# byteowlz/kokorox

Hardware: AMD Instinct MI355X
Metric: real-time factor (audio-s/wall-s), 24 kHz, batch=64 (higher is better)
Workload: dtype f32 in / out, f32 accumulate; products on split operands: f16f8 (a_hi b_hi on f16 MFMAs, the cross terms a_lo b_hi + a_hi b_lo of the 7 / 11-tap convs on e4m3 scaled MFMAs: ~17 significant bits per product; every other conv f16x3: ~22) -- wider than the bf16 BASELINE configs[2] names, inside the 1e-; 1 GPU; batch=64/GPU synthetic 128-phoneme utterances (T=130), durations pinned 3,3,3,4 -> F=422 frames = 10.55 s each, noise on, inputs in HBM; batch_per_gpu=64, frames=422, parallelism=utterance-sharded x1, one-time weight broadcast

## Files before the change

kokorox_amd/build.py:

```python
from __future__ import annotations

import os
import subprocess
import sys

HERE = os.path.dirname(os.path.abspath(__file__))
CSRC = os.path.join(HERE, "csrc")
LIB_DIR = os.path.join(HERE, "lib")
LIB_PATH = os.path.join(LIB_DIR, "libkokorox_hip.so")
TEST_LIB_PATH = os.path.join(LIB_DIR, "libkokorox_hip_test.so")
TEST_SOURCES = ["test_hooks.hip"]
SOURCES = ["conv_plan.hip", "conv_mfma.hip", "conv_f16x3.hip", "conv_f16x3_da.hip", "conv_f16x3_da_p1.hip", "conv_f16x3_da_w2.hip", "conv_f16x3_da_s16.hip", "conv_f16x3_da_f8.hip", "conv_f16x3_da_pre.hip", "conv_f16x3_pre.hip", "conv_f16x3_dapn.hip", "conv_f16x3_dag.hip", "kernels_misc.hip", "model.hip", "api.hip", "dispatcher.hip", "onnx_import.cpp"]
HEADERS = ["kx_common.h", "kx_error.h", "conv_epilogue.h", "conv_f16x3_common.h"]
_PUB = os.path.join("..", "..", "include", "kokorox_hip.h")
_PUB_TEST = os.path.join("..", "..", "include", "kokorox_hip_test.h")
EXTRA_DEPS = {"model.hip": ["onnx_import.h", "model.h", _PUB], "api.hip": ["model.h", "kx_handle.h", "api_guard.h", _PUB],
              "dispatcher.hip": ["model.h", "kx_handle.h", "dispatcher_core.h", _PUB],
              "test_hooks.hip": ["model.h", "kx_handle.h", "api_guard.h", _PUB, _PUB_TEST], "onnx_import.cpp": ["onnx_import.h"], "conv_f16x3_da_p1.hip": ["conv_f16x3_da.hip"], "conv_f16x3_da_w2.hip": ["conv_f16x3_da.hip"], "conv_f16x3_da_s16.hip": ["conv_f16x3_da.hip"], "conv_f16x3_da_f8.hip": ["conv_f16x3_da.hip"], "conv_f16x3_da_pre.hip": ["conv_f16x3_da.hip"]}
FLAGS = ["-O3", "--offload-arch=gfx950", "-fPIC", "-std=c++17", "-Wall", "-Wno-unused-result"]


def _hipcc() -> str:
    for cand in (os.environ.get("HIPCC"), "/opt/rocm/bin/hipcc", "hipcc"):
        if cand and (os.path.isabs(cand) and os.path.exists(cand) or not os.path.isabs(cand)):
            return cand
    return "hipcc"


def _newer(target: str, deps) -> bool:
    if not os.path.exists(target):
        return False
    t = os.path.getmtime(target)
    return all(os.path.getmtime(d) <= t for d in deps)


LAST_BUILD = {"compiled": [], "reused": [], "linked": False}


def build_library(force: bool = False, verbose: bool = False) -> str:
    LAST_BUILD["compiled"], LAST_BUILD["reused"], LAST_BUILD["linked"] = [], [], False
    os.makedirs(LIB_DIR, exist_ok=True)
    hdrs = [os.path.join(CSRC, h) for h in HEADERS]
    objs, test_objs, jobs = [], [], []
    for src in SOURCES + TEST_SOURCES:
        s = os.path.join(CSRC, src)
        o = os.path.join(LIB_DIR, os.path.splitext(src)[0] + ".o")
        (test_objs if src in TEST_SOURCES else objs).append(o)
        if force or not _newer(o, [s] + hdrs + [os.path.join(CSRC, d) for d in EXTRA_DEPS.get(src, [])]):
            flags = [f for f in FLAGS if not f.startswith("--offload-arch")] if src.endswith(".cpp") else FLAGS
            jobs.append([_hipcc(), *flags, "-c", s, "-o", o])
            LAST_BUILD["compiled"].append(src)
        else:
            LAST_BUILD["reused"].append(src)
    if jobs:
        from concurrent.futures import ThreadPoolExecutor

        def run(cmd):
            if verbose:
                print(" ".join(cmd), file=sys.stderr)
            subprocess.run(cmd, check=True)

        with ThreadPoolExecutor(max_workers=min(4, len(jobs))) as ex:
            list(ex.map(run, jobs))
    if force or not _newer(LIB_PATH, objs):
        cmd = [_hipcc(), "--offload-arch=gfx950", "-shared", "-fPIC", *objs, "-lpthread", "-o", LIB_PATH]
        if verbose:
            print(" ".join(cmd), file=sys.stderr)
        subprocess.run(cmd, check=True)
        LAST_BUILD["linked"] = True
    if force or not _newer(TEST_LIB_PATH, test_objs + [LIB_PATH]):
        cmd = [_hipcc(), "--offload-arch=gfx950", "-shared", "-fPIC", *test_objs, "-L" + LIB_DIR, "-lkokorox_hip", "-Wl,-rpath,$ORIGIN",
               "-lpthread", "-o", TEST_LIB_PATH]
        if verbose:
            print(" ".join(cmd), file=sys.stderr)
        subprocess.run(cmd, check=True)
    return LIB_PATH


if __name__ == "__main__":
    print(build_library(force="--force" in sys.argv, verbose=True))
```

kokorox_amd/csrc/conv_f16x3.hip:

```cpp
#include "conv_f16x3_common.h"

namespace kx {

template <int BM, int BN, int WM, int WN, int ACT, int TK, bool PF, int VT>
__global__ __launch_bounds__(WM * WN * 64, (WM * WN == 8) ? 4 : ((BM / WM / 32) * (BN / WN / 32) > 6 ? 2 : 3))
void conv1d_f16x3_kernel(const ConvArgs a) {
    constexpr int MT = BM / WM / 32;
    constexpr int NT = BN / WN / 32;
    constexpr int NWV = WM * WN;
    static_assert((NWV == 4 || NWV == 8) && MT >= 1 && NT >= 1, "4 or 8 waves per workgroup");
    static_assert(VT == 1 || (VT <= TK && PF), "virtual taps need TK >= VT and the prefetching build");
    extern __shared__ __attribute__((aligned(16))) unsigned char smem16[];

    const int tid = threadIdx.x;
    const int lane = tid & 63;
    const int wave = __builtin_amdgcn_readfirstlane(tid >> 6);
    const int wm = wave / WN, wn = wave % WN;
    const int r = lane & 31, h = lane >> 5;
    const int b = blockIdx.z, ct = blockIdx.y;
    int tile_x = blockIdx.x;
    if (a.xcd_swizzle && gridDim.x >= 16) {
        const int nx = gridDim.x;
        const int off = (int)(((long)nx * (blockIdx.y + (long)gridDim.y * blockIdx.z)) & 7);
        const int cls = (blockIdx.x + off) & 7;
// ... 223 lines not shown
                half8 al_[2][MT], bh[2][NT], ah[MT], bl[NT];
                load_P(0, al_[0], bh[0]);
#pragma unroll
                for (int tt = 0; tt < TK; ++tt) {
                    if (tt < taps) {
                        load_Q(tt, ah, bl);
#pragma unroll
                        for (int mt = 0; mt < MT; ++mt)
#pragma unroll
                            for (int nt = 0; nt < NT; ++nt)
                                acc[mt][nt] = __builtin_amdgcn_mfma_f32_32x32x16_f16(al_[tt & 1][mt], bh[tt & 1][nt], acc[mt][nt], 0, 0, 0);
                        if (tt + 1 < TK && tt + 1 < taps) load_P(tt + 1, al_[(tt + 1) & 1], bh[(tt + 1) & 1]);
#pragma unroll
                        for (int mt = 0; mt < MT; ++mt)
#pragma unroll
                            for (int nt = 0; nt < NT; ++nt) {
                                acc[mt][nt] = __builtin_amdgcn_mfma_f32_32x32x16_f16(ah[mt], bl[nt], acc[mt][nt], 0, 0, 0);
                                acc[mt][nt] = __builtin_amdgcn_mfma_f32_32x32x16_f16(ah[mt], bh[tt & 1][nt], acc[mt][nt], 0, 0, 0);
                            }
                    }
                }
            }
            unsigned long long tp0 = 0;
            if (a.stamps) tp0 = __builtin_amdgcn_s_memrealtime();
            if (pc + 1 == n_pieces && more)
                asm volatile("s_waitcnt lgkmcnt(0)\n\ts_barrier" ::: "memory");
            else
                __syncthreads();
            if (a.stamps) acc_pbar += __builtin_amdgcn_s_memrealtime() - tp0;
            cur ^= 1;
        }
        if (more) {
            unsigned long long ta = 0, tb = 0;
            if (a.stamps) ta = __builtin_amdgcn_s_memrealtime();
            if (!(a.dbg & 1)) stage_chunk(ch + 1, true);
            if (a.stamps) tb = __builtin_amdgcn_s_memrealtime();
            __syncthreads();
            if (a.stamps) {
                acc_stage += tb - ta;
                acc_bar += __builtin_amdgcn_s_memrealtime() - tb;
            }
        }
    }

    if (a.stamps) st2 = __builtin_amdgcn_s_memrealtime();
    if (a.dbg & 8) return;
    float2* stat_scr = (BM >= 64 || PF) ? reinterpret_cast<float2*>(smem16) + wave * (32 * 33) : nullptr;
    conv_store_tile<MT, NT, EPI_ROWS, (VT > 1)>(a, acc, a.w_unscale, b, ct * BM + wm * (MT * 32), t0 + wn * (NT * 32), r, h, ncols, Lout,
                            tile_x * WN + wn, stat_scr);
    if (a.stamps && tid == 0) {
        const unsigned lin = blockIdx.x + gridDim.x * (blockIdx.y + gridDim.y * blockIdx.z);
        unsigned long long* o = a.stamps + (unsigned long long)lin * 8;
        o[0] = st0; o[1] = st1; o[2] = st2;
        __builtin_amdgcn_s_waitcnt(0);
        o[3] = __builtin_amdgcn_s_memrealtime();
        o[4] = __builtin_amdgcn_s_getreg(63492);
        o[5] = __builtin_readcyclecounter() - cyc0;
        o[6] = acc_stage;
        o[7] = acc_bar | (acc_pbar << 32);
    }
}

int conv16_cu_count() {
    if (const int part = cu_count_override()) return part;
    static std::atomic<int> n[KX_MAX_DEVICES];
    int dev = 0;
    KX_HIP(hipGetDevice(&dev));
    if (dev < 0 || dev >= KX_MAX_DEVICES) return 256;
    int v = n[dev].load(std::memory_order_relaxed);
    if (v == 0) {
        hipDeviceProp_t pr;
        KX_HIP(hipGetDeviceProperties(&pr, dev));
        v = pr.multiProcessorCount > 0 ? pr.multiProcessorCount : 256;
        n[dev].store(v, std::memory_order_relaxed);
    }
    return v;
}

template <int BM, int BN, int WM, int WN, int ACT, int TK, bool PF, int VT = 1>
static void launch_inst16_pf(const ConvArgs& a, int B, int max_cols, hipStream_t s) {
    static DynLdsLimit lds_limit;
    auto kern = conv1d_f16x3_kernel<BM, BN, WM, WN, ACT, TK, PF, VT>;
    const int XW = (BN - 1) * a.stride + (a.K - 1) * a.dil + 1;
    const int XWp = PF ? ((VT > 1) ? 128 : BN + 128) : ((XW + 3) & ~3);
    KX_REQUIRE(!PF || (a.stride == 1 && XW <= XWp), "conv1d f16x3: the prefetching build needs stride 1 and a window <= BN + 128");
    const size_t lds = 16 * ((size_t)2 * TK * 4 * BM + (size_t)VT * 4 * XWp);
    KX_REQUIRE(lds <= 160 * 1024, "conv1d f16x3: LDS tile too large for this k/stride");
    KX_REQUIRE(VT == 1 || (a.K == 1 && a.stride == 1 && XW <= 128), "conv1d f16x3: virtual taps need a k=1 GEMM");
    lds_limit.ensure(reinterpret_cast<const void*>(kern), lds);
    dim3 grid((max_cols + BN - 1) / BN, (a.Cout + BM - 1) / BM, a.merge_T > 0 ? 1 : B);
    KX_REQUIRE(grid.x > 0 && grid.y > 0 && grid.y < 65536 && B > 0 && B < 65536, "conv1d f16x3: bad grid");
    KX_REQUIRE(a.merge_T == 0 || (PF && a.K == 1 && a.stride == 1 && a.pad == 0 && !a.in_up2 && !a.nmean &&
                                  a.store != ST_UPSCATTER && !a.stat_part),
               "conv1d f16x3: merged columns need a plain k=1 GEMM");
    hipLaunchKernelGGL(kern, grid, dim3(WM * WN * 64), lds, s, a);
    KX_HIP(hipGetLastError());
}

template <int BM, int BN, int WM, int WN, int ACT>
static void launch_inst16_act(const ConvPlan& p, const ConvArgs& a, int B, hipStream_t s) {
    if (p.pf)
        launch_inst16_pf<BM, BN, WM, WN, ACT, 3, true>(a, B, p.cols, s);
    else
        launch_inst16_pf<BM, BN, WM, WN, ACT, 3, false>(a, B, p.cols, s);
}

template <int BM, int BN, int WM, int WN>
static void launch_inst16(const ConvPlan& p, const ConvArgs& a, int B, hipStream_t s) {
    if (p.act == ACT_SNAKE)
        launch_inst16_act<BM, BN, WM, WN, ACT_SNAKE>(p, a, B, s);
    else if (p.act == ACT_LEAKY)
        launch_inst16_act<BM, BN, WM, WN, ACT_LEAKY>(p, a, B, s);
    else
        launch_inst16_act<BM, BN, WM, WN, ACT_NONE>(p, a, B, s);
}

static void launch_lds(const ConvPlan& p, const ConvArgs& a, int B, hipStream_t s) {
    if (p.vt > 1) {
        KX_REQUIRE(p.bm == 128 && p.bn == 128 && p.pf && p.act != ACT_SNAKE && (p.vt == 2 || p.vt == 3), "conv1d f16x3: no such virtual-tap form");
        if (p.vt == 3) {
            if (p.act == ACT_LEAKY)
                launch_inst16_pf<128, 128, 2, 2, ACT_LEAKY, 3, true, 3>(a, B, p.cols, s);
            else
                launch_inst16_pf<128, 128, 2, 2, ACT_NONE, 3, true, 3>(a, B, p.cols, s);
        } else {
            if (p.act == ACT_LEAKY)
                launch_inst16_pf<128, 128, 2, 2, ACT_LEAKY, 2, true, 2>(a, B, p.cols, s);
            else
                launch_inst16_pf<128, 128, 2, 2, ACT_NONE, 2, true, 2>(a, B, p.cols, s);
        }
        return;
    }
    const int bm = p.bm, bn = p.bn, wm = p.wm, wn = p.wn;
    if (bm == 128 && bn == 128 && wm == 4 && wn == 1)
        launch_inst16<128, 128, 4, 1>(p, a, B, s);
    else if (bm == 128 && bn == 128 && wm == 2 && wn == 2)
        launch_inst16<128, 128, 2, 2>(p, a, B, s);
    else if (bm == 128 && bn == 256 && wm == 2 && wn == 2)
        launch_inst16<128, 256, 2, 2>(p, a, B, s);
    else if (bm == 64 && bn == 256 && wm == 1 && wn == 4)
        launch_inst16<64, 256, 1, 4>(p, a, B, s);
    else if (bm == 32 && bn == 256 && wm == 1 && wn == 4)
        launch_inst16<32, 256, 1, 4>(p, a, B, s);
    else
        throw Error(1, "conv1d f16x3: no such LDS-DMA form");
}

void launch_conv(const ConvPlan& p, const ConvArgs& a, int B, hipStream_t s) {
    if (p.form == FORM_F32) {
        launch_conv1d(a, p.bm, B, p.cols, s);
        return;
    }
    KX_REQUIRE(a.n_chunks16 == (a.Cin + CK16 - 1) / CK16 && a.w16 != nullptr, "conv1d f16x3: weights not packed");
    KX_REQUIRE(a.epi != EPI_GELU_NEW || p.vt > 1 || p.form == FORM_DAG || p.form == FORM_DAGN,
               "conv1d f16x3: gelu epilogue exists only for k=1 GEMMs with >= 48 input channels");
    KX_REQUIRE(p.merged == (a.merge_T > 0), "conv1d f16x3: merged columns do not match the plan");
    if (p.cols <= 0) return;
    switch (p.form) {
        case FORM_LDS: launch_lds(p, a, B, s); return;
        case FORM_DAG:
        case FORM_DAGN: launch_conv1d_f16x3_dag(p, a, B, s); return;
        case FORM_DAPN: launch_conv1d_f16x3_dapn(a, B, p.cols, s); return;
        case FORM_DA_PRE: launch_conv16_da_pre(p, a, B, s); return;
        case FORM_DA_S16: launch_conv16_da_s16(p, a, B, s); return;
        case FORM_DA_F8: launch_conv16_da_f8(p, a, B, s); return;
        case FORM_DA:
            if (p.p1) {
                launch_conv16_da_p1(p, a, B, s);
                return;
            }
            [[fallthrough]];
        case FORM_DA_W2: {
            static const int dephase = getenv("KX_DEPHASE") ? atoi(getenv("KX_DEPHASE")) : 0;
            static const int dephase_mode = getenv("KX_DEPHASE_MODE") ? atoi(getenv("KX_DEPHASE_MODE")) : 1;
            ConvArgs d;
            const ConvArgs* ap = &a;
            if (dephase > 0 && p.bn == 256) {
                d = a;
                const long grid_n = (long)((p.cols + 255) / 256) * ((a.Cout + 127) / 128) * B;
                const double tile_cycles = (double)a.n_chunks16 * a.K * 8 * 96 * 2.5 + 50000.0;
                d.dephase_cycles = grid_n >= 1024 ? (int)(tile_cycles * dephase / 1000.0) : 0;
                d.dephase_mode = dephase_mode;
                ap = &d;
            }
            if (p.form == FORM_DA_W2)
                launch_conv16_da_w2(p, *ap, B, s);
            else
                launch_conv16_da(p, *ap, B, s);
            return;
        }
    }
    throw Error(1, "conv1d: unknown kernel form");
}

size_t packed_conv16_halves(int rows, int Cin, int K, int BM) {
    const size_t tiles = (rows + BM - 1) / BM, chunks = (Cin + CK16 - 1) / CK16;
    return tiles * chunks * K * 4 * BM * 8;
}

__global__ void absmax_kernel(const float* p, long n, unsigned* out) {
    float m = 0.f;
    for (long i = blockIdx.x * (long)blockDim.x + threadIdx.x; i < n; i += (long)gridDim.x * blockDim.x)
        m = fmaxf(m, fabsf(p[i]));
    for (int o = 32; o > 0; o >>= 1) m = fmaxf(m, __shfl_down(m, o));
    if ((threadIdx.x & 63) == 0) atomicMax(out, __float_as_uint(m));
}

float device_absmax(const float* p, long n, hipStream_t s) {
    unsigned* d;
    KX_HIP(hipMalloc((void**)&d, 4));
    KX_HIP(hipMemsetAsync(d, 0, 4, s));
    const int blocks = (int)((n + 255) / 256 < 1024 ? (n + 255) / 256 : 1024);
    hipLaunchKernelGGL(absmax_kernel, dim3(blocks), dim3(256), 0, s, p, n, d);
    unsigned hbits = 0;
    KX_HIP(hipMemcpyAsync(&hbits, d, 4, hipMemcpyDeviceToHost, s));
    KX_HIP(hipStreamSynchronize(s));
    KX_HIP(hipFree(d));
    float f;
    memcpy(&f, &hbits, 4);
    return f;
}

int pick_weight_shift(float absmax) {
    if (!(absmax > 0.f) || !std::isfinite(absmax)) return 0;
    int e;
    frexpf(absmax, &e);
    int ws = 12 - e;
    if (ws < -8) ws = -8;
    if (ws > 24) ws = 24;
    return ws;
}

__global__ void pack_conv16_kernel(PackSrc src, _Float16* dst, int Cout, int Cin, int K, int BM, float wscale,
                                   long total_pairs) {
    const int n_chunks = (Cin + CK16 - 1) / CK16;
    for (long e = blockIdx.x * (long)blockDim.x + threadIdx.x; e < total_pairs; e += (long)gridDim.x * blockDim.x) {
        long q = e;
        const int j8 = q % 8; q /= 8;
        const int m = q % BM; q /= BM;
        const int hh = q % 2; q /= 2;
        const int tap = q % K; q /= K;
        const int ch = q % n_chunks; q /= n_chunks;
        const int co = (int)q * BM + m, ci = ch * CK16 + hh * 8 + j8;
        float v = 0.f;
        if (co < Cout && ci < Cin) {
            int rr = co;
            const float* p = src.p[0];
            if (rr >= src.rows[0]) { rr -= src.rows[0]; p = src.p[1];
                if (rr >= src.rows[1]) { rr -= src.rows[1]; p = src.p[2]; } }
            v = p[((long)rr * Cin + ci) * K + tap] * wscale;
        }
        const _Float16 hi = (_Float16)v;
        const _Float16 lo = (_Float16)(v - (float)hi);
        const long base = ((((long)q * n_chunks + ch) * K + tap) * 2) * 2 * BM * 8;
        dst[base + ((0 * 2 + hh) * (long)BM + m) * 8 + j8] = hi;
        dst[base + ((1 * 2 + hh) * (long)BM + m) * 8 + j8] = lo;
    }
}

void launch_pack_conv16(const PackSrc& src, void* dst, int Cout, int Cin, int K, int BM, float wscale, hipStream_t s) {
    const long total = (long)packed_conv16_halves(Cout, Cin, K, BM) / 2;
    const int blocks = (int)((total + 255) / 256 < 4096 ? (total + 255) / 256 : 4096);
    hipLaunchKernelGGL(pack_conv16_kernel, dim3(blocks), dim3(256), 0, s, src, static_cast<_Float16*>(dst), Cout, Cin, K,
                       BM, wscale, total);
    KX_HIP(hipGetLastError());
}

__global__ void pack_convT16_kernel(const float* w, _Float16* dst, int Cin, int Cout, int sd, int BM, float wscale,
                                    long total_pairs) {
    const int n_chunks = (Cin + CK16 - 1) / CK16;
    const int rows = sd * Cout, k = 2 * sd;
    for (long e = blockIdx.x * (long)blockDim.x + threadIdx.x; e < total_pairs; e += (long)gridDim.x * blockDim.x) {
        long q = e;
        const int j8 = q % 8; q /= 8;
        const int m = q % BM; q /= BM;
        const int hh = q % 2; q /= 2;
        const int tap = q % 2; q /= 2;
        const int ch = q % n_chunks; q /= n_chunks;
        const int row = (int)q * BM + m, ci = ch * CK16 + hh * 8 + j8;
        float v = 0.f;
        if (row < rows && ci < Cin) {
            const int sdiv = sd, co = row / sdiv, p = row % sdiv;
            v = w[((long)ci * Cout + co) * k + (tap == 0 ? p + sd : p)] * wscale;
        }
        const _Float16 hi = (_Float16)v;
        const _Float16 lo = (_Float16)(v - (float)hi);
        const long base = ((((long)q * n_chunks + ch) * 2 + tap) * 2) * 2 * BM * 8;
        dst[base + ((0 * 2 + hh) * (long)BM + m) * 8 + j8] = hi;
        dst[base + ((1 * 2 + hh) * (long)BM + m) * 8 + j8] = lo;
    }
}

__global__ void image_to_bf16_kernel(const _Float16* src, unsigned short* dst, long n_halves, int plane) {
    for (long e = blockIdx.x * (long)blockDim.x + threadIdx.x; e < n_halves; e += (long)gridDim.x * blockDim.x) {
        const long blk = e / (2 * plane), in_blk = e - blk * 2 * plane;
        if (in_blk >= plane) {
            dst[e] = 0;
            continue;
        }
        const float v = (float)src[e] + (float)src[e + plane];
        unsigned u = __float_as_uint(v);
        u += 0x7fffu + ((u >> 16) & 1u);
        dst[e] = (unsigned short)(u >> 16);
    }
}
void launch_image_to_bf16(const void* w16, void* dst, size_t n_halves, hipStream_t s) {
    const int plane = 2 * 128 * 8;
    const int blocks = (int)((n_halves + 255) / 256 < 4096 ? (n_halves + 255) / 256 : 4096);
    hipLaunchKernelGGL(image_to_bf16_kernel, dim3(blocks), dim3(256), 0, s, static_cast<const _Float16*>(w16), static_cast<unsigned short*>(dst),
                       (long)n_halves, plane);
    KX_HIP(hipGetLastError());
}

size_t packed_conv8x_bytes(int rows, int Cin, int K) {
// ... 46 lines not shown
```

kokorox_amd/csrc/conv_plan.hip:

```cpp
#include "kx_common.h"

namespace kx {

static bool da_eligible(int BM, int K, int dil, int stride, bool merged) {
    return BM == 128 && stride == 1 && !merged && (K - 1) * dil + 256 <= 384;
}

static bool f8_taps(int K, int dil) { return (K == 11 || K == 7 || K == 3) && (K - 1) * dil <= 64; }

static bool s16_shape(int BM, int K, int dil, int stride, int act, int n_chunks16, bool merged, int pmode) {
    const bool taps = K == 11 || (K == 7 && dil == 1) || (pmode == 2 && f8_taps(K, dil));
    return BM == 128 && stride == 1 && !merged && pmode != 1 && act == ACT_SNAKE && taps && (K - 1) * dil <= 64 && n_chunks16 >= 2 &&
           (n_chunks16 & 1) == 0;
}

bool conv16_f8_layer(int BM, int rows, int K, int n_chunks16) {
    return BM == 128 && f8_taps(K, 1) && (K != 3 || rows <= 256) && n_chunks16 >= 2 && (n_chunks16 & 1) == 0;
}

ConvPlan conv_plan(const ConvLaunch& c) {
    ConvPlan p{};
    p.bm = c.BM;
    p.act = c.act;
    p.vt = 1;
    p.cols = c.cols;
    const bool stats = c.stats && c.store == ST_NORMAL && !c.accum;
    auto set_stats = [&](int stat_cols) {
        if (!stats) return;
        p.stat_cols = stat_cols;
        p.stat_tiles = (p.cols + p.bn - 1) / p.bn * (p.bn / stat_cols);
    };
    if (c.mode == CONV_F32) {
        p.form = FORM_F32;
        p.bn = c.BM == 128 ? 128 : 256;
        set_stats(64);
        return p;
    }
    const int route = c.force & 3;
    const int pmode = c.prec1 ? 1 : (c.f8 ? 2 : 0);

    const bool pre_form = c.stride == 1 && c.K >= 2 && !c.in_up2 && c.act != ACT_SNAKE && !c.prec1 &&
                          da_eligible(c.BM, c.K, c.dil, c.stride, false);
    p.pre = (c.mode == CONV_F16X3 || c.mode == CONV_F16F8) && c.image && pre_form && (c.image == 2 || c.rows >= 512);

    p.merged = c.B > 1 && c.K == 1 && c.stride == 1 && c.pad == 0 && !c.in_up2 && !c.norm && c.store != ST_UPSCATTER && !c.stats &&
               c.merge_T > 0 && c.merge_T <= 512;
    if (p.merged) p.cols = c.B * c.merge_T;

    if (c.BM != 128) {
        p.form = FORM_LDS;
        p.bn = 256;
        p.wm = 1;
        p.wn = 4;
        p.pf = c.stride == 1 && (c.K - 1) * c.dil <= 128;
        set_stats(64);
        return p;
    }

    if (c.K == 1 && c.stride == 1 && !stats && !c.in_up2 && c.n_chunks16 >= 3 && c.act != ACT_SNAKE) {
        const long tiles = (long)((p.cols + 127) / 128) * ((c.rows + 127) / 128);
        if (route != FORCE_LDS && !c.norm && c.store != ST_UPSCATTER) {
            const long wgs = tiles * (p.merged ? 1 : c.B);
            const bool narrow_ok = (c.x_bs * c.B + 16L * c.x_ld) * 4 < (1L << 31);
            p.form = narrow_ok && 2 * wgs <= c.cus ? FORM_DAGN : FORM_DAG;
            p.bn = p.form == FORM_DAGN ? 32 : 128;
            return p;
        }
        p.form = FORM_LDS;
        p.bn = 128;
        p.wm = 2;
        p.wn = 2;
        p.pf = 1;
        p.vt = tiles > 2L * c.cus ? 2 : 3;
        return p;
    }

    const bool da = route != FORCE_LDS && da_eligible(c.BM, c.K, c.dil, c.stride, p.merged);
    const bool small = (long)((p.cols + 255) / 256) * ((c.rows + 127) / 128) * c.B < 256;
    if (route != FORCE_LDS && !(c.force & FORCE_NO_S16) && s16_shape(c.BM, c.K, c.dil, c.stride, c.act, c.n_chunks16, p.merged, pmode)) {
        p.form = pmode == 2 ? FORM_DA_F8 : FORM_DA_S16;
        p.kt = c.K;
        p.bn = small && route != FORCE_DA ? 128 : 192;
        set_stats(64);
    } else if (!da || (route != FORCE_DA && c.cols <= 160 && !stats)) {
        p.form = FORM_LDS;
        const bool short_seq = c.cols <= 160 && !stats;
        p.bn = !short_seq && !small ? 256 : 128;
        p.wm = !short_seq && small ? 4 : 2;
        p.wn = !short_seq && small ? 1 : 2;
        p.pf = c.stride == 1 && (c.K - 1) * c.dil <= 128;
        set_stats(p.bn / p.wn);
    } else {
        p.bn = small && route != FORCE_DA ? 128 : 256;
        set_stats(128);
        const bool w64 = (c.K - 1) * c.dil <= 64;
        if (p.pre) {
            const bool narrow = p.bn == 128 && !c.prec1 && c.rows % 32 == 0 && c.K <= 12 && c.epi == EPI_NONE &&
                                (c.store == ST_NORMAL || c.store == ST_UPSCATTER) && (long)c.n_chunks16 * c.K < 5000;
            p.form = narrow ? FORM_DAPN : FORM_DA_PRE;
            p.act = ACT_NONE;
            p.kt = c.K == 3 && w64 ? 3 : 0;
        } else {
            const bool unrolled = w64 && ((c.act == ACT_SNAKE && (c.K == 11 || c.K == 7 || c.K == 3)) || (c.act == ACT_LEAKY && c.K == 3));
            p.kt = unrolled ? c.K : 0;
            p.p1 = c.prec1 != 0;
            p.bf = c.prec1 == 2;
            p.form = unrolled && p.bn == 256 && !c.prec1 && !(c.force & FORCE_DA_4X1) ? FORM_DA_W2 : FORM_DA;
        }
    }
    const bool flat_form = p.form != FORM_LDS;
    p.flat_bn = flat_form && c.B > 1 && p.cols > 0 ? p.bn : 0;
    return p;
}

}
```

kokorox_amd/csrc/kernels_misc.hip:

```cpp
#include <cmath>

#include <atomic>

#include "kx_common.h"

namespace kx {

__device__ __forceinline__ int len_of(const LenMap& m, int b) { return m.lens[b] * m.mul + m.add; }

__global__ void vec_add_kernel(const float* a, const float* b, float* out, int n) {
    int i = blockIdx.x * blockDim.x + threadIdx.x;
    if (i < n) out[i] = a[i] + (b ? b[i] : 0.f);
}
void launch_vec_add(const float* a, const float* b, float* out, int n, hipStream_t s) {
    hipLaunchKernelGGL(vec_add_kernel, dim3((n + 255) / 256), dim3(256), 0, s, a, b, out, n);
    KX_HIP(hipGetLastError());
}

__global__ void transpose_whh_kernel(const float* w, float* out) {
    int i = blockIdx.x * blockDim.x + threadIdx.x;
    if (i < 1024 * 256) {
        int r = i / 256, k = i % 256;
        out[((k >> 2) * 1024 + r) * 4 + (k & 3)] = w[i];
    }
}
void launch_transpose_whh(const float* whh, float* out, hipStream_t s) {
    hipLaunchKernelGGL(transpose_whh_kernel, dim3(1024), dim3(256), 0, s, whh, out);
    KX_HIP(hipGetLastError());
}

__device__ __forceinline__ long checked_id(long id, int n_vocab, int b, int t, unsigned* bad) {
    if (id >= 0 && id < n_vocab) return id;
    if (bad) atomicCAS(bad, 0u, (((unsigned)b << 16) | (unsigned)t) + 1u);
    return id < 0 ? 0 : n_vocab - 1;
}

__global__ void albert_embed_kernel(const int64_t* ids, long ids_stride, const float* word, const float* type0,
                                    const float* pos, float* out, long bs, int ld, const int* lens, int n_vocab,
                                    unsigned* bad) {
    const int t = blockIdx.x, b = blockIdx.y, e = threadIdx.x;
    if (t >= lens[b]) return;
    const long id = checked_id(ids[b * ids_stride + t], n_vocab, b, t, e == 0 ? bad : nullptr);
    out[b * bs + (long)e * ld + t] = (word[id * 128 + e] + type0[e]) + pos[t * 128 + e];
}
void launch_albert_embed(const int64_t* ids, long ids_stride, const float* word, const float* type0,
                         const float* pos, float* out, long bs, int ld, const int* lens, int B, int Tmax,
                         int n_vocab, unsigned* bad_id, hipStream_t s) {
    hipLaunchKernelGGL(albert_embed_kernel, dim3(Tmax, B), dim3(128), 0, s, ids, ids_stride, word, type0, pos,
                       out, bs, ld, lens, n_vocab, bad_id);
    KX_HIP(hipGetLastError());
}

__global__ void embed_kernel(const int64_t* ids, long ids_stride, const float* table, int C, float* out, long bs,
                             int ld, const int* lens, int n_vocab, unsigned* bad) {
    const int t = blockIdx.x, b = blockIdx.y;
    if (t >= lens[b]) return;
    const long id = checked_id(ids[b * ids_stride + t], n_vocab, b, t, threadIdx.x == 0 ? bad : nullptr);
    for (int c = threadIdx.x; c < C; c += blockDim.x) out[b * bs + (long)c * ld + t] = table[id * C + c];
}
void launch_embed(const int64_t* ids, long ids_stride, const float* table, int C, float* out, long bs, int ld,
                  const int* lens, int B, int Tmax, int n_vocab, unsigned* bad_id, hipStream_t s) {
    hipLaunchKernelGGL(embed_kernel, dim3(Tmax, B), dim3(256), 0, s, ids, ids_stride, table, C, out, bs, ld, lens,
                       n_vocab, bad_id);
    KX_HIP(hipGetLastError());
}

template <int CPT>
__global__ __launch_bounds__(1024) void layernorm_ch_kernel(const float* x, float* y, long bs, int ld, int C,
                                                            LenMap len, float eps, int mode, const float* g,
                                                            const float* be, int g_bs, float leaky) {
    __shared__ float red[2][16][16];
    const int tx = threadIdx.x & 15, cg = threadIdx.x >> 4, wave = threadIdx.x >> 6;
    const bool wave_lead = (threadIdx.x & 63) < 16;
    const int b = blockIdx.y, t = blockIdx.x * 16 + tx;
    const int L = len_of(len, b);
    const bool ok = t < L;
    const float* xb = x + b * bs + (ok ? t : 0);
    float v[CPT];
    float s = 0.f;
#pragma unroll
    for (int i = 0; i < CPT; ++i) {
        const int c = cg + 64 * i;
        v[i] = (ok && c < C) ? xb[(long)c * ld] : 0.f;
        s += v[i];
    }
    s += __shfl_xor(s, 16);
    s += __shfl_xor(s, 32);
    if (wave_lead) red[0][wave][tx] = s;
    __syncthreads();
    float tot = 0.f;
#pragma unroll
    for (int k = 0; k < 16; ++k) tot += red[0][k][tx];
    const float mean = tot / (float)C;
    float q = 0.f;
#pragma unroll
    for (int i = 0; i < CPT; ++i) {
        const int c = cg + 64 * i;
        const float d = (c < C) ? v[i] - mean : 0.f;
        q += d * d;
    }
    q += __shfl_xor(q, 16);
    q += __shfl_xor(q, 32);
    if (wave_lead) red[1][wave][tx] = q;
    __syncthreads();
    float qt = 0.f;
#pragma unroll
    for (int k = 0; k < 16; ++k) qt += red[1][k][tx];
    const float rstd = 1.0f / sqrtf(qt / (float)C + eps);
    if (!ok) return;
    float* yb = y + b * bs + t;
#pragma unroll
    for (int i = 0; i < CPT; ++i) {
        const int c = cg + 64 * i;
        if (c >= C) continue;
        float o = (v[i] - mean) * rstd;
        if (mode == LN_AFFINE)
            o = o * g[c] + be[c];
        else if (mode == LN_ADA)
            o = (1.0f + g[(long)b * g_bs + c]) * o + be[(long)b * g_bs + c];
        if (leaky != 0.f) o = o > 0.f ? o : o * leaky;
        yb[(long)c * ld] = o;
    }
}
void launch_layernorm_ch(const float* x, float* y, long bs, int ld, int C, LenMap len, int B, int Lmax, float eps,
                         int mode, const float* g, const float* be, int g_bs, float leaky, hipStream_t s) {
    if (Lmax <= 0) return;
    KX_REQUIRE(C <= 768, "layernorm: at most 768 channels");
    const dim3 grid((Lmax + 15) / 16, B), block(1024);
    if (C <= 128)
        hipLaunchKernelGGL(layernorm_ch_kernel<2>, grid, block, 0, s, x, y, bs, ld, C, len, eps, mode, g, be, g_bs, leaky);
    else if (C <= 512)
        hipLaunchKernelGGL(layernorm_ch_kernel<8>, grid, block, 0, s, x, y, bs, ld, C, len, eps, mode, g, be, g_bs, leaky);
    else
        hipLaunchKernelGGL(layernorm_ch_kernel<12>, grid, block, 0, s, x, y, bs, ld, C, len, eps, mode, g, be, g_bs, leaky);
    KX_HIP(hipGetLastError());
}

__global__ __launch_bounds__(256) void attention_mfma_kernel(const float* qkv, long bs, int ld, float* ctx, long cbs,
                                                             int cld, const int* lens) {
    using f32x16 = __attribute__((ext_vector_type(16))) float;
    const int b = blockIdx.x, hd = blockIdx.y;
    const int lane = threadIdx.x & 63, wave = threadIdx.x >> 6;
    const int i = lane & 31, hh = lane >> 5;
    const int T = lens[b];
    const int q0 = (blockIdx.z * 4 + wave) * 32;
    if (q0 >= T) return;
    const float* Q = qkv + b * bs + (long)(hd * 64) * ld;
    const float* Kp = Q + (long)768 * ld;
    const float* V = Q + (long)1536 * ld;
    const int qi = q0 + i < T ? q0 + i : T - 1;
    float qreg[32];
#pragma unroll
    for (int s = 0; s < 32; ++s) qreg[s] = Q[(long)(2 * s + hh) * ld + qi];
    f32x16 o0, o1;
#pragma unroll
    for (int e = 0; e < 16; ++e) o0[e] = o1[e] = 0.f;
    float mrun = -INFINITY, lrun = 0.f;
    for (int k0 = 0; k0 < T; k0 += 32) {
        const int kj = k0 + i < T ? k0 + i : T - 1;
        f32x16 st;
#pragma unroll
        for (int e = 0; e < 16; ++e) st[e] = 0.f;
#pragma unroll
        for (int s = 0; s < 32; ++s)
            st = __builtin_amdgcn_mfma_f32_32x32x2f32(Kp[(long)(2 * s + hh) * ld + kj], qreg[s], st, 0, 0, 0);
        float bm = -INFINITY;
#pragma unroll
        for (int e = 0; e < 16; ++e) {
            const int j = k0 + (e & 3) + 8 * (e >> 2) + 4 * hh;
            st[e] = j < T ? st[e] * 0.125f : -INFINITY;
            bm = fmaxf(bm, st[e]);
        }
        bm = fmaxf(bm, __shfl_xor(bm, 32));
        const float mn = fmaxf(mrun, bm);
        const float alpha = expf(mrun - mn);
        float psum = 0.f;
#pragma unroll
        for (int e = 0; e < 16; ++e) {
            st[e] = expf(st[e] - mn);
            psum += st[e];
        }
        psum += __shfl_xor(psum, 32);
        lrun = lrun * alpha + psum;
        mrun = mn;
#pragma unroll
        for (int e = 0; e < 16; ++e) {
            o0[e] *= alpha;
            o1[e] *= alpha;
        }
#pragma unroll
        for (int dt = 0; dt < 2; ++dt) {
            const float* vrow = V + (long)(dt * 32 + i) * ld + k0 + 4 * hh;
            float vv[16];
#pragma unroll
            for (int g4 = 0; g4 < 4; ++g4) {
                const float4 v4 = *reinterpret_cast<const float4*>(vrow + 8 * g4);
                const int j = k0 + 8 * g4 + 4 * hh;
                vv[4 * g4 + 0] = j + 0 < T ? v4.x : 0.f;
                vv[4 * g4 + 1] = j + 1 < T ? v4.y : 0.f;
                vv[4 * g4 + 2] = j + 2 < T ? v4.z : 0.f;
                vv[4 * g4 + 3] = j + 3 < T ? v4.w : 0.f;
            }
#pragma unroll
            for (int s = 0; s < 16; ++s) {
                if (dt == 0)
                    o0 = __builtin_amdgcn_mfma_f32_32x32x2f32(vv[s], st[s], o0, 0, 0, 0);
                else
                    o1 = __builtin_amdgcn_mfma_f32_32x32x2f32(vv[s], st[s], o1, 0, 0, 0);
            }
        }
    }
    if (q0 + i < T) {
        const float inv = 1.0f / lrun;
        float* cb = ctx + b * cbs + (long)(hd * 64) * cld + q0 + i;
#pragma unroll
        for (int e = 0; e < 16; ++e) {
            const int d = (e & 3) + 8 * (e >> 2) + 4 * hh;
            cb[(long)d * cld] = o0[e] * inv;
            cb[(long)(32 + d) * cld] = o1[e] * inv;
        }
    }
}

void launch_attention(const float* qkv, long bs, int ld, float* ctx, long cbs, int cld, const int* lens, int B,
                      int Tmax, hipStream_t s) {
    KX_REQUIRE(Tmax <= 512, "attention: T > 512");
    KX_REQUIRE(ld % 32 == 0 && ld >= ((Tmax + 31) & ~31), "attention: rows must be padded to a multiple of 32 columns");
    hipLaunchKernelGGL(attention_mfma_kernel, dim3(B, 12, (Tmax + 127) / 128), dim3(256), 0, s, qkv, bs, ld, ctx, cbs,
                       cld, lens);
    KX_HIP(hipGetLastError());
}

__global__ __launch_bounds__(256) void style_fc_kernel(const FcDesc* desc, const float* styles, float* out,
                                                       long out_bs) {
    __shared__ float sv[128];
    const FcDesc d = desc[blockIdx.x];
    const int b = blockIdx.y;
    if (threadIdx.x < 128) sv[threadIdx.x] = styles[b * 256 + d.style_off + threadIdx.x];
    __syncthreads();
    for (int o = threadIdx.x; o < d.n_out; o += 256) {
        const float4* wr = reinterpret_cast<const float4*>(d.w + (long)o * 128);
        float acc = 0.f;
#pragma unroll 8
        for (int k = 0; k < 32; ++k) {
            const float4 w4 = wr[k];
            acc += w4.x * sv[4 * k] + w4.y * sv[4 * k + 1] + w4.z * sv[4 * k + 2] + w4.w * sv[4 * k + 3];
        }
        out[b * out_bs + d.out_off + o] = acc + d.b[o];
    }
}
__global__ void tile_prefix_kernel(LenMap len, int extra, int bn, int B, int* out) {
    if (threadIdx.x != 0 || blockIdx.x != 0) return;
    int acc = 0;
    for (int b = 0; b < B; ++b) {
        out[b] = acc;
        const int cols = len.lens[b] * len.mul + len.add + extra;
        acc += cols > 0 ? (cols + bn - 1) / bn : 0;
    }
    out[B] = acc;
}

void launch_tile_prefix(LenMap len, int extra, int bn, int B, int* out, hipStream_t s) {
    hipLaunchKernelGGL(tile_prefix_kernel, dim3(1), dim3(64), 0, s, len, extra, bn, B, out);
    KX_HIP(hipGetLastError());
}

void launch_style_fc(const FcDesc* d_desc, int n_desc, const float* styles, float* out, long out_bs, int B,
                     hipStream_t s) {
    hipLaunchKernelGGL(style_fc_kernel, dim3(n_desc, B), dim3(256), 0, s, d_desc, styles, out, out_bs);
    KX_HIP(hipGetLastError());
}

__global__ __launch_bounds__(256) void in_stats_kernel(const float* x, long bs, int ld, LenMap len, const float* gb,
                                                       long gb_bs, int C, float* mean, float* scale, float* shift,
                                                       int n_bs, float2* raw_out) {
    __shared__ double rs[4], rq[4];
    const int c = blockIdx.x, b = blockIdx.y;
    const int L = len_of(len, b);
    const float* row = x + b * bs + (long)c * ld;
    double s = 0.0, q = 0.0;
    const int L4 = L & ~3;
    const float4* row4 = reinterpret_cast<const float4*>(row);
    int t = threadIdx.x;
    for (; 4 * (t + 256) < L4; t += 512) {
        const float4 u = row4[t], w = row4[t + 256];
        const double a0 = u.x, a1 = u.y, a2 = u.z, a3 = u.w, b0 = w.x, b1 = w.y, b2 = w.z, b3 = w.w;
        s += ((a0 + a1) + (a2 + a3)) + ((b0 + b1) + (b2 + b3));
        q += ((a0 * a0 + a1 * a1) + (a2 * a2 + a3 * a3)) + ((b0 * b0 + b1 * b1) + (b2 * b2 + b3 * b3));
    }
    for (; 4 * t < L4; t += 256) {
        const float4 u = row4[t];
        const double a0 = u.x, a1 = u.y, a2 = u.z, a3 = u.w;
        s += (a0 + a1) + (a2 + a3);
        q += (a0 * a0 + a1 * a1) + (a2 * a2 + a3 * a3);
    }
    for (int e = L4 + threadIdx.x; e < L; e += 256) {
        const double v = (double)row[e];
        s += v;
        q += v * v;
    }
    for (int o = 32; o > 0; o >>= 1) {
        s += __shfl_down(s, o);
        q += __shfl_down(q, o);
    }
    const int lane = threadIdx.x & 63, wave = threadIdx.x >> 6;
    if (lane == 0) {
        rs[wave] = s;
        rq[wave] = q;
    }
    __syncthreads();
    if (threadIdx.x == 0) {
        const double S = (rs[0] + rs[1]) + (rs[2] + rs[3]), Q = (rq[0] + rq[1]) + (rq[2] + rq[3]);
        if (raw_out) {
            const float sh = (float)S, qh = (float)Q;
            raw_out[((long)b * C + c) * 2 + 0] = make_float2(sh, qh);
            raw_out[((long)b * C + c) * 2 + 1] = make_float2((float)(S - (double)sh), (float)(Q - (double)qh));
        }
        const double m = L > 0 ? S / L : 0.0;
        double var = L > 0 ? Q / L - m * m : 0.0;
        if (var < 0.0) var = 0.0;
        const float rstd = (float)(1.0 / sqrt(var + 1e-5));
        const float g = gb[b * gb_bs + c], be = gb[b * gb_bs + C + c];
        mean[(long)b * n_bs + c] = (float)m;
        scale[(long)b * n_bs + c] = (1.0f + g) * rstd;
        shift[(long)b * n_bs + c] = be;
    }
}
void launch_in_stats(const float* x, long bs, int ld, int C, LenMap len, int B, const float* gb, long gb_bs,
                     float* mean, float* scale, float* shift, int n_bs, float2* raw_out, hipStream_t s) {
    hipLaunchKernelGGL(in_stats_kernel, dim3(C, B), dim3(256), 0, s, x, bs, ld, len, gb, gb_bs, C, mean, scale,
                       shift, n_bs, raw_out);
    KX_HIP(hipGetLastError());
}

__global__ __launch_bounds__(64) void stats_finalize_kernel(const float2* part, int tiles, int cols_per_tile, int C,
                                                            LenMap len, const float* gb, long gb_bs, float* mean,
                                                            float* scale, float* shift, int n_bs) {
    const int c = blockIdx.x, b = blockIdx.y;
    const int L = len_of(len, b);
    const int used = ((L + cols_per_tile - 1) / cols_per_tile);
    const float2* p = part + ((long)b * C + c) * tiles;
    double s = 0.0, q = 0.0;
    for (int i = threadIdx.x; i < used && i < tiles; i += 64) {
        const float2 v = p[i];
        s += (double)v.x;
        q += (double)v.y;
    }
    for (int o = 32; o > 0; o >>= 1) {
        s += __shfl_down(s, o);
        q += __shfl_down(q, o);
    }
    if (threadIdx.x == 0) {
        const double m = L > 0 ? s / L : 0.0;
        double var = L > 0 ? q / L - m * m : 0.0;
        if (var < 0.0) var = 0.0;
        const float rstd = (float)(1.0 / sqrt(var + 1e-5));
        const float g = gb[b * gb_bs + c], be = gb[b * gb_bs + C + c];
        mean[(long)b * n_bs + c] = (float)m;
        scale[(long)b * n_bs + c] = (1.0f + g) * rstd;
        shift[(long)b * n_bs + c] = be;
    }
}
void launch_stats_finalize(const float2* part, int tiles, int cols_per_tile, int C, LenMap len, int B, const float* gb,
                           long gb_bs, float* mean, float* scale, float* shift, int n_bs, hipStream_t s) {
    hipLaunchKernelGGL(stats_finalize_kernel, dim3(C, B), dim3(64), 0, s, part, tiles, cols_per_tile, C, len, gb, gb_bs,
                       mean, scale, shift, n_bs);
    KX_HIP(hipGetLastError());
}

__global__ void style_mix_kernel(const float* table, int n_voices, const int* voice_ids, const float* weights,
                                 int max_mix, const int* rows, const int* kinds, float* styles) {
#pragma clang fp contract(off)
    const int b = blockIdx.x, j = threadIdx.x;
    const int kind = kinds ? kinds[b] : (max_mix == 1 ? 1 : 2);
    if (kind == 0) return;
    const int row = rows[b];
    const int* v = voice_ids + (long)b * max_mix;
    const float* w = weights + (long)b * max_mix;
    float acc = 0.f;
    if (kind == 1) {
        acc = table[((long)v[0] * 511 + row) * 256 + j];
    } else {
// ... 776 lines not shown
```

kokorox_amd/csrc/kx_common.h:

```cpp
#pragma once
#include <hip/hip_runtime.h>

#include <cmath>
#include <cstdint>
#include <cstring>
#include <cstdio>
#include <stdexcept>
#include <string>

#include <atomic>
#include <mutex>

#include "kx_error.h"

namespace kx {

constexpr int KX_MAX_DEVICES = 64;

struct DynLdsLimit {
    std::atomic<size_t> limit[KX_MAX_DEVICES];
    std::mutex mu;
    DynLdsLimit() {
        for (auto& l : limit) l.store(64 * 1024);
    }
    void ensure(const void* kern, size_t lds) {
        int dev = 0;
        if (hipGetDevice(&dev) != hipSuccess || dev < 0 || dev >= KX_MAX_DEVICES) throw Error(3, "dynamic LDS limit: bad current device");
        if (lds <= limit[dev].load(std::memory_order_acquire)) return;
        std::lock_guard<std::mutex> lk(mu);
        if (lds <= limit[dev].load(std::memory_order_relaxed)) return;
        const hipError_t e = hipFuncSetAttribute(kern, hipFuncAttributeMaxDynamicSharedMemorySize, (int)lds);
        if (e != hipSuccess) throw Error(3, std::string("hipFuncSetAttribute(MaxDynamicSharedMemorySize): ") + hipGetErrorString(e));
        limit[dev].store(lds, std::memory_order_release);
    }
};

#define KX_HIP(expr)                                                                       \
    do {                                                                                   \
        hipError_t e_ = (expr);                                                            \
        if (e_ != hipSuccess)                                                              \
            throw kx::Error(3, std::string(#expr) + ": " + hipGetErrorString(e_) + " (" +  \
                                   __FILE__ + ":" + std::to_string(__LINE__) + ")");       \
    } while (0)

#define KX_REQUIRE(cond, msg)                                 \
    do {                                                      \
        if (!(cond)) throw kx::Error(1, std::string(msg));    \
    } while (0)

struct LenMap {
    const int* lens;
    int mul, add;
};

constexpr int CONV_CK = 8;

enum ConvAct { ACT_NONE = 0, ACT_LEAKY = 1, ACT_SNAKE = 2 };
enum ConvStore { ST_NORMAL = 0, ST_TMAJOR = 1, ST_UPSCATTER = 2 };
enum ConvEpi { EPI_NONE = 0, EPI_GELU_NEW = 1 };

struct ConvArgs {
    const float* x;
    long x_bs;
    int x_ld;
    int Cin;
    LenMap in_len;
    LenMap out_len;
    const float* w;
    const float* bias;
    const float* nmean;
    const float* nscale;
    const float* nshift;
    int n_bs;
    int act;
    float slope;
    const float* alpha;
    int K, dil, stride, pad;
    int in_up2;
    int Cout;
    int n_chunks;
    float* y;
    long y_bs;
    int y_ld;
    const float* resid;
    long r_bs;
    int r_ld;
    int accum;
    float out_mul;
    float out_div;
    int epi;
    int store;
    int up_s, up_pad, up_off, up_reflect, up_cout;
    const void* w16;
    const void* w16b;
    const void* w8x;
    int epi_stream;
    int n_chunks16;
    float w_unscale;
    float x_prescale;
    int merge_T;
    int merge_B;
    float2* stat_part;
    int stat_tiles;
    int xcd_swizzle;
    int ws_force;
    unsigned long long* stamps;
    int prec1;
    int dephase_cycles, dephase_mode;
    int dbg;
    const int* tile_prefix;
    int flat_ny;
    int flat_B;
    int flat_tiles_host, flat_bn_host;
    const void* x16;
    long x16_bs;
    int x16_ld;
};

enum ConvMode { CONV_F32 = 0, CONV_F16X3 = 1, CONV_F16X3_LDS = 2, CONV_F16X3_DA = 3, CONV_F16 = 4, CONV_BF16 = 5, CONV_F16F8 = 6 };
enum ConvForm {
    FORM_F32 = 0,
    FORM_LDS,
    FORM_DAG,
    FORM_DAGN,
    FORM_DA,
    FORM_DA_W2,
    FORM_DA_S16,
    FORM_DA_F8,
    FORM_DA_PRE,
    FORM_DAPN,
};
enum ConvForce { FORCE_LDS = 1, FORCE_DA = 2, FORCE_DA_4X1 = 4, FORCE_NO_S16 = 8 };

struct ConvLaunch {
    int mode;
    int prec1;
    int f8;
    int BM, rows, n_chunks16, K, dil, stride, pad, act, in_up2, store, accum, epi;
    int norm;
    int stats;
    int image;
    int merge_T;
    long x_bs;
    int x_ld;
    int B, cols;
    int cus;
    int force;
};
struct ConvPlan {
    int form;
    int bm, act, kt, wm, wn, vt, pf, p1, bf;
    int bn;
    int cols;
    int merged;
    int pre;
    int stat_cols, stat_tiles;
    int flat_bn;
};
ConvPlan conv_plan(const ConvLaunch& c);
bool conv16_f8_layer(int BM, int rows, int K, int n_chunks16);
void launch_conv(const ConvPlan& p, const ConvArgs& a, int B, hipStream_t s);
int conv16_cu_count();
int cu_count_override();

size_t conv16_pre_image_bytes(int Cin, int x_ld);
void launch_split_image(const ConvArgs& a, int B, int Lmax, void* img, long img_bs, hipStream_t s);

void launch_tile_prefix(LenMap len, int extra, int bn, int B, int* out, hipStream_t s);

inline int conv_pick_bm(int rows) { return rows >= 128 ? 128 : (rows > 32 ? 64 : 32); }

void launch_conv1d(const ConvArgs& a, int BM, int B, int max_cols, hipStream_t s);

struct PackSrc {
    const float* p[3];
    int rows[3];
};
void launch_pack_conv(const PackSrc& src, float* dst, int Cout, int Cin, int K, int BM, hipStream_t s);
void launch_pack_convT(const float* w, float* dst, int Cin, int Cout, int s, int BM, hipStream_t s_);
size_t packed_conv_floats(int rows, int Cin, int K, int BM);

void launch_conv16_da(const ConvPlan& p, const ConvArgs& a, int B, hipStream_t s);
void launch_conv16_da_p1(const ConvPlan& p, const ConvArgs& a, int B, hipStream_t s);
void launch_conv16_da_w2(const ConvPlan& p, const ConvArgs& a, int B, hipStream_t s);
void launch_conv16_da_s16(const ConvPlan& p, const ConvArgs& a, int B, hipStream_t s);
void launch_conv16_da_f8(const ConvPlan& p, const ConvArgs& a, int B, hipStream_t s);
void launch_conv16_da_pre(const ConvPlan& p, const ConvArgs& a, int B, hipStream_t s);
void launch_conv1d_f16x3_dapn(const ConvArgs& a, int B, int max_cols, hipStream_t s);
void launch_conv1d_f16x3_dag(const ConvPlan& p, const ConvArgs& a, int B, hipStream_t s);
size_t packed_conv16_halves(int rows, int Cin, int K, int BM);
float device_absmax(const float* p, long n, hipStream_t s);
int pick_weight_shift(float absmax);
void launch_pack_conv16(const PackSrc& src, void* dst, int Cout, int Cin, int K, int BM, float wscale, hipStream_t s);
void launch_pack_convT16(const float* w, void* dst, int Cin, int Cout, int sd, int BM, float wscale, hipStream_t s);
void launch_image_to_bf16(const void* w16, void* dst, size_t n_halves, hipStream_t s);
size_t packed_conv8x_bytes(int rows, int Cin, int K);
void launch_pack_conv8x(const void* w16, void* dst, int rows, int Cin, int K, hipStream_t s);

void launch_vec_add(const float* a, const float* b, float* out, int n, hipStream_t s);
void launch_transpose_whh(const float* whh, float* out, hipStream_t s);

void launch_albert_embed(const int64_t* ids, long ids_stride, const float* word, const float* type0,
                         const float* pos, float* out, long bs, int ld, const int* lens, int B, int Tmax,
                         int n_vocab, unsigned* bad_id, hipStream_t s);
void launch_embed(const int64_t* ids, long ids_stride, const float* table, int C, float* out, long bs, int ld,
                  const int* lens, int B, int Tmax, int n_vocab, unsigned* bad_id, hipStream_t s);

enum LnMode { LN_PLAIN = 0, LN_AFFINE = 1, LN_ADA = 2 };
void launch_layernorm_ch(const float* x, float* y, long bs, int ld, int C, LenMap len, int B, int Lmax,
                         float eps, int mode, const float* g, const float* be, int g_bs, float leaky,
                         hipStream_t s);

void launch_attention(const float* qkv, long bs, int ld, float* ctx, long cbs, int cld, const int* lens, int B,
                      int Tmax, hipStream_t s);

struct FcDesc {
    const float* w;
    const float* b;
    int n_out;
    int style_off;
    long out_off;
};
void launch_style_fc(const FcDesc* d_desc, int n_desc, const float* styles, float* out, long out_bs, int B,
                     hipStream_t s);

void launch_stats_finalize(const float2* part, int tiles, int cols_per_tile, int C, LenMap len, int B, const float* gb,
                           long gb_bs, float* mean, float* scale, float* shift, int n_bs, hipStream_t s);
void launch_in_stats(const float* x, long bs, int ld, int C, LenMap len, int B, const float* gb, long gb_bs,
                     float* mean, float* scale, float* shift, int n_bs, float2* raw_out, hipStream_t s);

void launch_diag_stats(const float* x, long bs, int ld, int C, LenMap len, int B, int Lmax, const float* nmean,
                       const float* nscale, const float* nshift, int n_bs, float* out3, hipStream_t s);

void launch_style_mix(const float* table, int n_voices, const int* voice_ids, const float* weights, int max_mix,
                      const int* rows, const int* kinds, float* styles, int B, hipStream_t s);
void launch_pack_audio(const float* audio, long audio_ld, const int* frames, int B, int Fmax, int format, void* out,
                       long out_stride_bytes, const long* out_off, hipStream_t s, const int* formats = nullptr);
void* host_out_alloc(size_t bytes);
void host_out_free(void* p);
void host_out_share(void* base, void* const* parts, int n);
size_t host_out_live_bytes();
void launch_fill_style_rows(float* dst, long bs, int ld, int row0, const float* styles, int style_off,
                            const int* lens, int B, int Tmax, hipStream_t s);
void launch_copy_rows(const float* src, long sbs, int sld, float* dst, long dbs, int dld, int rows, LenMap len,
                      int B, int Lmax, hipStream_t s);

void launch_lstm(const float* gx, long gx_bs, int gx_ld, const float* whhT, float* y, long y_bs, int y_ld,
                 LenMap len, int B, unsigned long long* xchg, unsigned* err_word, hipStream_t s,
                 unsigned* epoch_state = nullptr);
size_t lstm_exchange_bytes(int B);
void lstm_set_parts(int n);
void lstm_set_test_fault(int on);

void launch_duration(const float* logits, long bs, int ld, const float* speeds, int n_speed, const int* lens,
                     const int* pinned, int n_pinned, int* dur, int* frames, int* idx, int idx_ld, int B,
                     hipStream_t s);
void launch_gather_cols(const float* src, long sbs, int sld, float* dst, long dbs, int dld, int C,
                        const int* idx, int idx_ld, const int* frames, int B, int Fmax, hipStream_t s);

void launch_pool_up2(const float* x, long xbs, int xld, int C, const float* mean, const float* scale,
                     const float* shift, int n_bs, float slope, const float* w, const float* bias, float* y,
                     long ybs, int yld, LenMap in_len, int B, int Lmax_in, hipStream_t s);

void launch_source(const float* f0, long f0_bs, const int* frames, int B, int Fmax, const float* lin_w,
                   const float* lin_b, uint64_t seed, uint64_t utt_base, const uint64_t* utt_seeds, int noise_off,
                   float* phase_ws,
                   float* har, long har_bs, hipStream_t s);
enum StftVariant { STFT_ONNX = 0, STFT_TORCH = 1 };
void launch_stft(const float* har_src, long hs_bs, float* har, long bs, int ld, const int* frames, int B,
                 int Fmax, int variant, hipStream_t s);
void launch_istft_head(const float* cp, long bs, int ld, float* spec_ws, float* audio, long audio_ld,
                       const int* frames, int B, int Fmax, int variant, hipStream_t s);
void init_dft_tables();

}
```

kokorox_amd/csrc/model.h:

```cpp
#pragma once
#include <atomic>
#include <map>
#include <mutex>
#include <string>
#include <vector>

#include "kx_common.h"

namespace kx {

struct TensorInfo {
    size_t offset = 0, nbytes = 0;
    int ndim = 0;
    int dims[4] = {0, 0, 0, 0};
};

struct ConvW {
    const float* w = nullptr;
    const float* bias = nullptr;
    int rows = 0, Cin = 0, K = 0, BM = 0, n_chunks = 0;
    int up_s = 0, up_cout = 0;
    const void* w16 = nullptr;
    const void* w16b = nullptr;
    const void* w8x = nullptr;
    int n_chunks16 = 0;
    float unscale = 1.f;
    std::string name;
    int act_shift = 0;
};

struct LstmW {
    ConvW ih;
    const float* whhT = nullptr;
};

struct Arena {
    char* base = nullptr;
    size_t cap = 0, off = 0;
    bool measure = false;
    void* alloc(size_t bytes) {
        const size_t a = (off + 255) & ~size_t(255);
        off = a + bytes;
        if (measure) return nullptr;
        if (off > cap) throw Error(3, "arena overflow (internal sizing bug)");
        return base + a;
    }
    float* f(size_t n) { return static_cast<float*>(alloc(n * sizeof(float))); }
    int* i(size_t n) { return static_cast<int*>(alloc(n * sizeof(int))); }
};

struct Tap {
    std::vector<float> data;
    int B = 0, C = 0, ld = 0;
    std::vector<int> L;
};

struct T {
    float* p = nullptr;
    long bs = 0;
    int ld = 0;
    int C = 0;
    LenMap len{nullptr, 1, 0};
    int Lmax = 0;
    T rows(int r0, int n) const {
        T t = *this;
        t.p = p + (long)r0 * ld;
        t.C = n;
        return t;
    }
};

struct ConvOpts {
    const float* nmean = nullptr;
    const float* nscale = nullptr;
    const float* nshift = nullptr;
    int act = ACT_NONE;
    float slope = 0.f;
    const float* alpha = nullptr;
    int dil = 1, stride = 1, pad = 0, in_up2 = 0;
    const T* resid = nullptr;
    int accum = 0;
    float out_mul = 1.f, out_div = 1.f;
    int epi = EPI_NONE;
    int store = ST_NORMAL;
    int up_pad = 0, up_off = 0, up_reflect = 0;
    LenMap up_len{nullptr, 1, 0};
    float2* stat_part = nullptr;
};

std::vector<unsigned char> read_weight_file(const char* path, int* variant = nullptr);
std::vector<unsigned char> import_onnx_bytes(const unsigned char* data, size_t n, int* variant = nullptr);

struct LstmTimeout : Error {
    explicit LstmTimeout(const std::string& m) : Error(3, m) {}
};

class Model {
  public:
    Model(int device, int part = 0, int n_parts = 1);
    ~Model();
    void load_file(const char* path);
    void load_device_blob(const void* d_blob, size_t n, bool adopt = false);
    void adopt_blob_guard(void* d_blob) { blob_ = static_cast<char*>(d_blob); }

    void infer_device(const int64_t* d_ids, int64_t t_stride, const int32_t* lens_host, int B,
                      const float* d_styles, const float* speeds_host, int n_speed, uint64_t seed, uint32_t flags,
                      float* d_audio, int64_t audio_ld, int32_t* d_frames, int64_t* need_ld);
    void infer_host(const int64_t* ids, int64_t t_stride, const int32_t* lens, int B, const float* styles,
                    const float* speeds, int n_speed, uint64_t seed, uint32_t flags, float** out,
                    int64_t* out_lens, const uint64_t* utt_seeds = nullptr);
    struct HostCall {
        const float* styles = nullptr;
        const int32_t* voice_ids = nullptr;
        const float* weights = nullptr;
        int max_mix = 0;
        const uint64_t* utt_seeds = nullptr;
        int format = 0;
        const int32_t* kinds = nullptr;
        const int32_t* formats = nullptr;
    };
    void infer_host_ex(const int64_t* ids, int64_t t_stride, const int32_t* lens, int B, const float* speeds,
                       int n_speed, uint64_t seed, uint32_t flags, const HostCall& hc, void** out, int64_t* out_bytes,
                       int64_t* out_samples);
    void status(int64_t out[4]) const;
    void note_clean_forward();
    void note_rerun() { n_rerun_ += 1; }
    static constexpr int LSTM_REARM_AFTER = 64;
    void set_voice_table(const float* table, int n_voices);
    int n_voices() const { return n_voices_.load(std::memory_order_acquire); }
    int n_vocab() const { return n_vocab_; }
    void sync();
    void order_after_null_stream();
    void order_null_stream_after();
    void set_pinned(const int32_t* pattern, int n);
    void warmup(int B, int n_tokens, int frames_per_token);
    void arena_bytes(int64_t out[3]) const { out[0] = (int64_t)arenaT_.cap; out[1] = (int64_t)arenaF_.cap; out[2] = (int64_t)arenaIO_.cap; }
    void call_times(double out[4]) const { for (int i = 0; i < 4; ++i) out[i] = call_ms_[i]; }
    void profile_enable(bool on);
    void profile_read(int64_t* launches, double* ms, double* flops);
    struct ProfRec { int rows, Cin, K, dil, stride, store; double cols, flops; float ms; double bytes; };
    void profile_aux(int64_t* stats_launches, double* stats_bytes);
    std::vector<ProfRec> prof_detail;
    struct DiagRec { std::string name; int rows, Cin, K, act_shift; double absmax, rms, count; };
    void diag_enable(bool on);
    const std::vector<DiagRec>& diag_collect();
    void set_act_shift(const std::string& conv_name, int shift);
    int get_act_shift(const std::string& conv_name) const;
    const Tap* find_tap(const std::string& name) const;

    int cu_partition(int* n_parts) const { *n_parts = n_parts_; return part_; }
    void info(int64_t out[8]) const;
    void set_source_variant(int v) { source_variant_ = v; }
    std::mutex mu;
    uint64_t utt_base = 0;
    void set_lanes(int n) { lanes_cfg_ = n < 0 ? 0 : (n > N_LANES ? N_LANES : n); }
    void set_conv_mode(int mode);
    int conv_mode = CONV_F16F8;
    int stft_variant = STFT_ONNX;
    int device;

  private:
    void build();
    const float* wt(const std::string& name) const;
    const TensorInfo& info(const std::string& name) const;
    bool has(const std::string& name) const { return table_.count(name) != 0; }
    float* dev_alloc(size_t floats);
    void pack16(ConvW& c, const PackSrc& src, const float* wT, int n_src_floats[3]);
    ConvW make_conv(const std::string& name, bool bias = true);
    ConvW make_conv_cat(const std::vector<std::string>& names);
    ConvW make_convT(const std::string& name, int stride);
    LstmW make_lstm(const std::string& name);
    void add_fc(const std::string& key, const std::string& fc_name, int style_off);
    long fc_off(const std::string& key) const;

    void conv(const ConvW& w, const T& in, const T& out, const ConvOpts& o);
    void stats(const T& x, const std::string& fc_key);
    void adain_resblk(const std::string& name, const T& x, const T& out, bool upsample, float* ws_a, float* ws_b,
                      float* ws_c);
    void adain_resblock1(const std::string& name, int k, const T& x, const T& xj, const T& t1, const T& out,
                         int accum, float out_div, float2* part_t1, float2* part_xj, hipEvent_t wait_before_last = nullptr);
    void lstm(const LstmW& w, const T& in, const T& out, float* gx);
    void tap(const char* name, const T& t);
    void ensure_arena(Arena& a, size_t bytes);

    static constexpr int N_LANES = 4;
    struct Lane {
        hipStream_t stream = nullptr;
        float *nmean = nullptr, *nscale = nullptr, *nshift = nullptr;
    };
    Lane lanes_[N_LANES];
    int lanes_cfg_ = 0;
    int n_lanes_ = 1;
    std::vector<hipEvent_t> lane_ev_;
    size_t lane_ev_used_ = 0;
    hipEvent_t record_here();
    void wait_here(hipEvent_t e);
    struct LaneScope;
    struct DeviceTurn;
    void sync_lanes();

    int part_ = 0, n_parts_ = 1, cu_count_ = 0;
    int source_variant_ = -2;
    std::vector<uint32_t> cu_mask_;
    void new_stream(hipStream_t* s);
    hipStream_t stream_ = nullptr;
    hipStream_t stream2_ = nullptr;
    hipEvent_t ev_fork_ = nullptr, ev_join_ = nullptr;
    char* blob_ = nullptr;
    size_t blob_bytes_ = 0;
    std::map<std::string, TensorInfo> table_;
    std::vector<void*> owned_;
    std::map<std::string, ConvW> convs_;
    std::map<std::string, LstmW> lstms_;
    std::vector<FcDesc> fc_host_;
    std::map<std::string, long> fc_off_;
    FcDesc* fc_dev_ = nullptr;
    long gb_total_ = 0;
    int n_vocab_ = 178;

    Arena arenaT_, arenaF_, arenaIO_;
    const uint64_t* d_utt_seeds_ = nullptr;
    float* d_voices_ = nullptr;
    std::atomic<int> n_voices_{0};
    int* d_pinned_ = nullptr;
    Arena* stats_arena_ = nullptr;
    Arena* img_arena_ = nullptr;
    int n_pinned_ = 0;

    int B_ = 0, Tmax_ = 0, Fmax_ = 0;
    std::vector<int> hT_, hF_;
    int *dT_ = nullptr, *dF_ = nullptr;
    unsigned long long* d_xchg_[2] = {nullptr, nullptr};
    size_t xchg_cap_ = 0;
    unsigned xchg_epoch_[2] = {0, 0};
    bool p1_region_ = false;
    bool lstm_pair_ok_ = true;
    int lstm_rearm_in_ = 0;
    int64_t n_lstm_timeouts_ = 0, n_rerun_ = 0;
    void infer_host_once(const int64_t* ids, int64_t t_stride, const int32_t* lens, int B, const float* speeds, int n_speed,
                         uint64_t seed, uint32_t flags, const HostCall& hc, void** out, int64_t* out_bytes, int64_t* out_samples);
    std::vector<long> h_off_;
    unsigned h_bad_id_ = 0;
    unsigned* d_dev_err_ = nullptr;
    unsigned* h_words_ = nullptr;
    int* h_stage_ = nullptr;
    size_t h_stage_cap_ = 0;
    int* stage_ints(size_t n);
    hipEvent_t ev_null_ = nullptr;
    hipEvent_t ev_done_ = nullptr;
    hipStream_t main_stream_ = nullptr;
    void check_dev_err();
    unsigned* d_bad_id_ = nullptr;
    float* gb_ = nullptr;
    float *nmean_ = nullptr, *nscale_ = nullptr, *nshift_ = nullptr;
    int n_bs_ = 0;
    bool taps_on_ = false;
    bool dry_ = false;
    std::map<std::string, Tap> taps_;

    struct PrefixKey { const int* lens; int mul, add, bn; hipStream_t stream; const int* dev; };
    std::vector<PrefixKey> prefix_keys_;
    int* d_prefix_ = nullptr;
    size_t prefix_cap_ = 0, prefix_used_ = 0;
    const int* tile_prefix_for(const LenMap& lm, int extra, int bn, int* total);

    struct PartInfo { const float2* part; int tiles, cols_per_tile, C; };
    std::map<const float*, PartInfo> parts_;

    double call_ms_[4] = {0, 0, 0, 0};
    bool diag_on_ = false;
    std::vector<DiagRec> diag_recs_;
    float* d_diag_ = nullptr;
    size_t diag_cap_ = 0, diag_used_ = 0;
    bool prof_on_ = false;
    std::vector<hipEvent_t> ev_;
    size_t ev_used_ = 0;
    double prof_flops_ = 0.0;
    std::vector<ProfRec> prof_recs_;
    int64_t prof_launches_ = 0;
    int64_t prof_stats_launches_ = 0;
    double prof_stats_bytes_ = 0.0;
};

}
```

kokorox_amd/csrc/model.hip:

```cpp
#include <chrono>
#include "model.h"

#include <sys/stat.h>
#include <unistd.h>

#include <cstdlib>
#include <cstring>

#include "onnx_import.h"

namespace kx {

static constexpr float RSQRT2 = 0.70710678118654752f;
static inline int up4(int x) { return (x + 31) & ~31; }

static thread_local int tl_cu_override = 0;
int cu_count_override() { return tl_cu_override; }
struct CuScope {
    int saved;
    explicit CuScope(int n) : saved(tl_cu_override) { tl_cu_override = n; }
    ~CuScope() { tl_cu_override = saved; }
};

Model::Model(int dev, int part, int n_parts) : device(dev), part_(part), n_parts_(n_parts) {
// ... 369 lines not shown
    c.bias = bias;
    float* wh = dev_alloc(2 * 256 * 1024);
    launch_transpose_whh(wt(name + ".weight_hh_l0"), wh, stream_);
    launch_transpose_whh(wt(name + ".weight_hh_l0_reverse"), wh + 256 * 1024, stream_);
    l.whhT = wh;
    return l;
}

void Model::add_fc(const std::string& key, const std::string& fc_name, int style_off) {
    const TensorInfo& ti = info(fc_name + ".weight");
    KX_REQUIRE(ti.dims[1] == 128, "style fc: expected 128 inputs");
    FcDesc d;
    d.w = wt(fc_name + ".weight");
    d.b = wt(fc_name + ".bias");
    d.n_out = ti.dims[0];
    d.style_off = style_off;
    d.out_off = gb_total_;
    fc_off_[key] = gb_total_;
    gb_total_ += d.n_out;
    fc_host_.push_back(d);
}
long Model::fc_off(const std::string& key) const {
    auto it = fc_off_.find(key);
    if (it == fc_off_.end()) throw Error(4, "internal: unknown style fc " + key);
    return it->second;
}

void Model::build() {
    {
        const TensorInfo& we = info("bert.embeddings.word_embeddings.weight");
        const TensorInfo& te = info("text_encoder.embedding.weight");
        n_vocab_ = we.dims[0] < te.dims[0] ? we.dims[0] : te.dims[0];
        KX_REQUIRE(n_vocab_ >= 1, "weight blob: empty embedding table");
    }
    const std::string L = "bert.encoder.albert_layer_groups.0.albert_layers.0.";
    convs_["bert.map"] = make_conv("bert.encoder.embedding_hidden_mapping_in");
    convs_["bert.qkv"] = make_conv_cat({L + "attention.query", L + "attention.key", L + "attention.value"});
    convs_["bert.dense"] = make_conv(L + "attention.dense");
    convs_["bert.ffn"] = make_conv(L + "ffn");
    convs_["bert.ffn_out"] = make_conv(L + "ffn_output");
    convs_["bert_encoder"] = make_conv("bert_encoder");
    for (int i = 0; i < 3; ++i) {
        const std::string n = "predictor.text_encoder.lstms." + std::to_string(2 * i);
        lstms_[n] = make_lstm(n);
        add_fc("dur_enc." + std::to_string(i), "predictor.text_encoder.lstms." + std::to_string(2 * i + 1) + ".fc", 128);
    }
    lstms_["predictor.lstm"] = make_lstm("predictor.lstm");
    lstms_["predictor.shared"] = make_lstm("predictor.shared");
    lstms_["text_encoder.lstm"] = make_lstm("text_encoder.lstm");
    convs_["duration_proj"] = make_conv("predictor.duration_proj.linear_layer");
    auto reg_resblk = [&](const std::string& n, int style_off) {
        convs_[n + ".conv1"] = make_conv(n + ".conv1");
        convs_[n + ".conv2"] = make_conv(n + ".conv2");
        if (has(n + ".conv1x1.weight")) convs_[n + ".conv1x1"] = make_conv(n + ".conv1x1", false);
        add_fc(n + ".norm1", n + ".norm1.fc", style_off);
        add_fc(n + ".norm2", n + ".norm2.fc", style_off);
    };
    for (const char* br : {"F0", "N"}) {
        for (int i = 0; i < 3; ++i) reg_resblk(std::string("predictor.") + br + "." + std::to_string(i), 128);
        convs_[std::string("predictor.") + br + "_proj"] = make_conv(std::string("predictor.") + br + "_proj");
    }
    for (int i = 0; i < 3; ++i)
        convs_["text_encoder.cnn." + std::to_string(i)] = make_conv("text_encoder.cnn." + std::to_string(i) + ".0");
    reg_resblk("decoder.encode", 0);
    for (int i = 0; i < 4; ++i) reg_resblk("decoder.decode." + std::to_string(i), 0);
    convs_["decoder.F0_conv"] = make_conv("decoder.F0_conv");
    convs_["decoder.N_conv"] = make_conv("decoder.N_conv");
    convs_["decoder.asr_res"] = make_conv("decoder.asr_res.0");
    const std::string G = "decoder.generator.";
    auto reg_resblock1 = [&](const std::string& n) {
        for (int i = 0; i < 3; ++i) {
            const std::string s = std::to_string(i);
            convs_[n + ".convs1." + s] = make_conv(n + ".convs1." + s);
            convs_[n + ".convs2." + s] = make_conv(n + ".convs2." + s);
            add_fc(n + ".adain1." + s, n + ".adain1." + s + ".fc", 0);
            add_fc(n + ".adain2." + s, n + ".adain2." + s + ".fc", 0);
        }
    };
    for (int i = 0; i < 2; ++i) {
        convs_[G + "noise_convs." + std::to_string(i)] = make_conv(G + "noise_convs." + std::to_string(i));
        reg_resblock1(G + "noise_res." + std::to_string(i));
    }
    convs_[G + "ups.0"] = make_convT(G + "ups.0", 10);
    convs_[G + "ups.1"] = make_convT(G + "ups.1", 6);
    for (int i = 0; i < 6; ++i) reg_resblock1(G + "resblocks." + std::to_string(i));
    convs_[G + "conv_post"] = make_conv(G + "conv_post");

    for (auto& kv : convs_) kv.second.name = kv.first;
    if (conv_mode == CONV_BF16 || conv_mode == CONV_F16F8) set_conv_mode(conv_mode);
    for (auto& kv : lstms_) kv.second.ih.name = kv.first + ".ih";
    KX_HIP(hipMalloc((void**)&fc_dev_, fc_host_.size() * sizeof(FcDesc)));
    owned_.push_back(fc_dev_);
    KX_HIP(hipMemcpyAsync(fc_dev_, fc_host_.data(), fc_host_.size() * sizeof(FcDesc), hipMemcpyHostToDevice, stream_));
    KX_HIP(hipStreamSynchronize(stream_));
}

void Model::ensure_arena(Arena& a, size_t bytes) {
    if (bytes <= a.cap) return;
    KX_HIP(hipStreamSynchronize(stream_));
    if (a.base) KX_HIP(hipFree(a.base));
    a.base = nullptr;
    a.cap = 0;
    const size_t want = bytes + bytes / 2 + (1 << 20);
    KX_HIP(hipMalloc((void**)&a.base, want));
    a.cap = want;
}



hipEvent_t Model::record_here() {
    if (dry_) return nullptr;
    if (lane_ev_used_ == lane_ev_.size()) {
        hipEvent_t e;
        KX_HIP(hipEventCreateWithFlags(&e, hipEventDisableTiming));
        lane_ev_.push_back(e);
    }
    hipEvent_t e = lane_ev_[lane_ev_used_++];
    KX_HIP(hipEventRecord(e, stream_));
    return e;
}

void Model::wait_here(hipEvent_t e) {
    if (dry_ || !e) return;
    KX_HIP(hipStreamWaitEvent(stream_, e, 0));
}

void Model::sync_lanes() {
    for (int i = 1; i < N_LANES; ++i)
        if (lanes_[i].stream) (void)hipStreamSynchronize(lanes_[i].stream);
}

struct Model::LaneScope {
    Model& m;
    hipStream_t s0;
    float *a0, *b0, *c0;
    LaneScope(Model& mm, int k) : m(mm), s0(mm.stream_), a0(mm.nmean_), b0(mm.nscale_), c0(mm.nshift_) {
        const Lane& L = m.lanes_[k < m.n_lanes_ ? k : 0];
        if (L.stream == m.stream_) return;
        hipEvent_t e = m.record_here();
        m.stream_ = L.stream;
        m.nmean_ = L.nmean;
        m.nscale_ = L.nscale;
        m.nshift_ = L.nshift;
        m.wait_here(e);
    }
    ~LaneScope() {
        m.stream_ = s0;
        m.nmean_ = a0;
        m.nscale_ = b0;
        m.nshift_ = c0;
    }
};

void Model::conv(const ConvW& w, const T& in, const T& out, const ConvOpts& o) {
    const int prec1 = (conv_mode == CONV_F16 && p1_region_) ? 1 : ((conv_mode == CONV_BF16 && p1_region_ && w.w16b) ? 2 : 0);
    const void* w8x = conv_mode == CONV_F16F8 ? w.w8x : nullptr;
    ConvLaunch c{};
    c.mode = conv_mode;
    c.prec1 = prec1;
    c.f8 = w8x != nullptr;
    c.BM = w.BM;
    c.rows = w.rows;
    c.n_chunks16 = w.n_chunks16;
    c.K = w.K;
    c.dil = o.dil;
    c.stride = o.stride;
    c.pad = o.pad;
    c.act = o.act;
    c.in_up2 = o.in_up2;
    c.store = o.store;
    c.accum = o.accum;
    c.epi = o.epi;
    c.norm = o.nmean != nullptr;
    c.stats = o.stat_part != nullptr;
    c.image = img_arena_ ? 1 : 0;
    const bool plain_lens = in.len.mul == 1 && in.len.add == 0 && out.len.lens == in.len.lens && out.len.mul == 1 && out.len.add == 0;
    c.merge_T = plain_lens ? in.Lmax : 0;
    c.x_bs = in.bs;
    c.x_ld = in.ld;
    c.B = B_;
    c.cols = (o.store == ST_UPSCATTER) ? in.Lmax + 1 : out.Lmax;
    c.cus = dry_ ? 0 : conv16_cu_count();
    const ConvPlan plan = conv_plan(c);
    void* x16 = nullptr;
    long x16_bs = 0;
    if (plan.pre) {
        x16_bs = (long)conv16_pre_image_bytes(w.Cin, in.ld);
        x16 = img_arena_->alloc((size_t)B_ * x16_bs);
    }
    if (dry_) return;
    ConvArgs a{};
    a.x = in.p;
    a.x_bs = in.bs;
    a.x_ld = in.ld;
    a.Cin = w.Cin;
    KX_REQUIRE(in.C == w.Cin, "internal: conv Cin mismatch");
    a.in_len = in.len;
    if (o.in_up2) {
        a.in_len.mul *= 2;
        a.in_len.add *= 2;
    }
    a.out_len = (o.store == ST_UPSCATTER) ? o.up_len : out.len;
    a.w = w.w;
    a.bias = w.bias;
    a.nmean = o.nmean;
    a.nscale = o.nscale;
    a.nshift = o.nshift;
    a.n_bs = n_bs_;
    a.act = o.act;
    a.slope = o.slope;
    a.alpha = o.alpha;
    a.K = w.K;
    a.dil = o.dil;
    a.stride = o.stride;
    a.pad = o.pad;
    a.in_up2 = o.in_up2;
    a.Cout = w.rows;
    a.n_chunks = w.n_chunks;
    a.y = out.p;
    a.y_bs = out.bs;
    a.y_ld = out.ld;
    if (o.resid) {
        a.resid = o.resid->p;
        a.r_bs = o.resid->bs;
        a.r_ld = o.resid->ld;
    }
    a.accum = o.accum;
    a.out_mul = o.out_mul;
    a.out_div = o.out_div;
    a.epi = o.epi;
    a.store = o.store;
    a.up_s = w.up_s;
    a.up_pad = o.up_pad;
    a.up_off = o.up_off;
    a.up_reflect = o.up_reflect;
    a.up_cout = w.up_cout ? w.up_cout : 1;
    const bool f16 = plan.form != FORM_F32;
    a.prec1 = prec1;
    a.w16 = w.w16;
    a.w16b = w.w16b;
    a.w8x = w8x;
    static const long stream_mb = getenv("KX_EPI_STREAM_MB") ? atol(getenv("KX_EPI_STREAM_MB")) : 512;
    a.epi_stream = f16 && stream_mb >= 0 && (double)B_ * w.rows * out.ld * 4.0 > (double)stream_mb * 1048576.0;
    a.n_chunks16 = w.n_chunks16;
    static const int xcd_swz = getenv("KX_XCD_SWIZZLE") ? atoi(getenv("KX_XCD_SWIZZLE")) : 1;
    a.xcd_swizzle = xcd_swz;
    a.x_prescale = std::ldexp(1.0f, w.act_shift);
    a.w_unscale = std::ldexp(w.unscale, -w.act_shift);
    if (diag_on_ && diag_used_ < diag_cap_) {
        float* slot = d_diag_ + 3 * diag_used_++;
        launch_diag_stats(in.p, in.bs, in.ld, w.Cin, in.len, B_, in.Lmax, o.nmean, o.nscale, o.nshift, n_bs_, slot, stream_);
        diag_recs_.push_back(DiagRec{w.name, w.rows, w.Cin, w.K, w.act_shift, 0.0, 0.0, 0.0});
    }
    parts_.erase(out.p);
    if (plan.stat_cols) {
        a.stat_part = o.stat_part;
        a.stat_tiles = plan.stat_tiles;
        parts_[out.p] = PartInfo{o.stat_part, a.stat_tiles, plan.stat_cols, w.rows};
    }
    static const int dbg_env = getenv("KX_DBG") ? atoi(getenv("KX_DBG")) : 0;
    a.dbg = dbg_env;
    const int max_cols = plan.cols;
    if (plan.merged) {
        a.merge_T = in.Lmax;
        a.merge_B = B_;
    }
    if (plan.flat_bn) {
        const LenMap& lm = (o.store == ST_UPSCATTER) ? a.in_len : a.out_len;
        const int extra = o.store == ST_UPSCATTER ? 1 : 0;
        int total = 0;
        a.tile_prefix = tile_prefix_for(lm, extra, plan.flat_bn, &total);
        a.flat_ny = (w.rows + 127) / 128;
        a.flat_B = B_;
        a.flat_tiles_host = total;
        a.flat_bn_host = plan.flat_bn;
        if (total <= 0) return;
    }
    static const char* stamp_path = getenv("KX_STAMP");
    static bool stamped = false;
    unsigned long long* d_stamps = nullptr;
    long n_wg = 0;
    static const int stamp_rows = getenv("KX_STAMP_ROWS") ? atoi(getenv("KX_STAMP_ROWS")) : 128;
    static const int stamp_k = getenv("KX_STAMP_K") ? atoi(getenv("KX_STAMP_K")) : 11;
    static int stamp_skip = getenv("KX_STAMP_SKIP") ? atoi(getenv("KX_STAMP_SKIP")) : 0;
    const bool stamp_match = stamp_path && !stamped && f16 && w.K == stamp_k && w.rows == stamp_rows && B_ >= 8 && !dry_;
    if (stamp_match && stamp_skip > 0) --stamp_skip;
    else if (stamp_match) {
        n_wg = (long)((max_cols + 127) / 128) * ((w.rows + 127) / 128) * (a.merge_T > 0 ? 1 : B_);
        KX_HIP(hipMalloc((void**)&d_stamps, n_wg * 64));
        KX_HIP(hipMemsetAsync(d_stamps, 0, n_wg * 64, stream_));
        a.stamps = d_stamps;
    }
    if (x16_bs) {
        launch_split_image(a, B_, in.Lmax, x16, x16_bs, stream_);
        a.x16 = x16;
        a.x16_bs = x16_bs;
        a.x16_ld = in.ld;
    }
    if (prof_on_ && w.BM == 128) {
        const LenMap& lm = (o.store == ST_UPSCATTER) ? in.len : out.len;
        const std::vector<int>& hl = (lm.lens == dT_) ? hT_ : hF_;
        double cols = 0;
        for (int b = 0; b < B_; ++b) cols += (double)hl[b] * lm.mul + lm.add + (o.store == ST_UPSCATTER ? 1 : 0);
        prof_flops_ += 2.0 * w.rows * w.Cin * w.K * cols;
        prof_launches_ += 1;
        double in_cols = 0;
        {
            const std::vector<int>& hi = (in.len.lens == dT_) ? hT_ : hF_;
            for (int b = 0; b < B_; ++b) in_cols += (double)hi[b] * in.len.mul + in.len.add;
        }
        const double out_rows = (o.store == ST_UPSCATTER) ? (double)(w.up_cout ? w.up_cout : 1) : (double)w.rows;
        const double out_cols = (o.store == ST_UPSCATTER) ? cols * w.up_s : cols;
        const double out_elems = out_rows * out_cols;
        const double bytes = 4.0 * ((double)w.Cin * in_cols + out_elems * (1.0 + (o.resid ? 1.0 : 0.0) + (o.accum ? 1.0 : 0.0)) +
                                    (double)w.rows * w.Cin * w.K);
        prof_recs_.push_back(ProfRec{w.rows, w.Cin, w.K, o.dil, o.stride, o.store, cols, 2.0 * w.rows * w.Cin * w.K * cols, 0.f, bytes});
        if (ev_used_ + 2 > ev_.size()) {
            for (int i = 0; i < 64; ++i) {
                hipEvent_t e;
                KX_HIP(hipEventCreate(&e));
                ev_.push_back(e);
            }
        }
        KX_HIP(hipEventRecord(ev_[ev_used_], stream_));
    }
    launch_conv(plan, a, B_, stream_);
    if (prof_on_ && w.BM == 128) {
        KX_HIP(hipEventRecord(ev_[ev_used_ + 1], stream_));
        ev_used_ += 2;
    }
    if (d_stamps) {
        stamped = true;
        KX_HIP(hipStreamSynchronize(stream_));
        std::vector<unsigned long long> hst(n_wg * 8);
        KX_HIP(hipMemcpy(hst.data(), d_stamps, n_wg * 64, hipMemcpyDeviceToHost));
        KX_HIP(hipFree(d_stamps));
        if (FILE* f = fopen(stamp_path, "wb")) {
            fwrite(hst.data(), 8, hst.size(), f);
            fclose(f);
        }
    }
}

const int* Model::tile_prefix_for(const LenMap& lm, int extra, int bn, int* total) {
    const std::vector<int>& hl = (lm.lens == dT_) ? hT_ : hF_;
    KX_REQUIRE(lm.lens == dT_ || lm.lens == dF_, "internal: tile prefix of an unknown length array");
    int tot = 0;
    for (int b = 0; b < B_; ++b) {
        const int cols = hl[b] * lm.mul + lm.add + extra;
        tot += cols > 0 ? (cols + bn - 1) / bn : 0;
    }
    *total = tot;
    for (const PrefixKey& k : prefix_keys_)
        if (k.lens == lm.lens && k.mul == lm.mul && k.add == lm.add + extra && k.bn == bn && k.stream == stream_) return k.dev;
    const size_t need = (size_t)(B_ + 1);
    if (prefix_used_ + need > prefix_cap_) {
        const size_t want = std::max<size_t>(prefix_cap_ * 2, (size_t)64 * need);
        int* p = nullptr;
        KX_HIP(hipMalloc((void**)&p, want * sizeof(int)));
        owned_.push_back(p);
        d_prefix_ = p;
        prefix_cap_ = want;
        prefix_used_ = 0;
    }
    int* dev = d_prefix_ + prefix_used_;
    prefix_used_ += need;
    launch_tile_prefix(lm, extra, bn, B_, dev, stream_);
    prefix_keys_.push_back(PrefixKey{lm.lens, lm.mul, lm.add + extra, bn, stream_, dev});
    return dev;
}

void Model::stats(const T& x, const std::string& fc_key) {
    float2* raw = stats_arena_ ? reinterpret_cast<float2*>(stats_arena_->alloc((size_t)B_ * x.C * 2 * sizeof(float2))) : nullptr;
    if (dry_) return;
    auto it = parts_.find(x.p);
    if (it != parts_.end() && it->second.C == x.C) {
        const PartInfo& pi = it->second;
        launch_stats_finalize(pi.part, pi.tiles, pi.cols_per_tile, x.C, x.len, B_, gb_ + fc_off(fc_key), gb_total_,
                              nmean_, nscale_, nshift_, n_bs_, stream_);
        return;
    }
    if (prof_on_) {
        const std::vector<int>& hl = (x.len.lens == dT_) ? hT_ : hF_;
        double cols = 0;
        for (int b = 0; b < B_; ++b) cols += (double)hl[b] * x.len.mul + x.len.add;
        prof_stats_bytes_ += 4.0 * x.C * cols;
        prof_stats_launches_ += 1;
    }
    launch_in_stats(x.p, x.bs, x.ld, x.C, x.len, B_, gb_ + fc_off(fc_key), gb_total_, nmean_, nscale_, nshift_, n_bs_,
                    raw, stream_);
    if (raw) parts_[x.p] = PartInfo{raw, 2, 1, x.C};
}

void Model::tap(const char* name, const T& t) {
    if (!taps_on_ || dry_) return;
    KX_HIP(hipStreamSynchronize(stream_));
    Tap tp;
    tp.B = B_;
    tp.C = t.C;
    tp.ld = t.ld;
    tp.data.resize((size_t)B_ * t.C * t.ld);
    const std::vector<int>& hl = (t.len.lens == dT_) ? hT_ : hF_;
    for (int b = 0; b < B_; ++b) {
        tp.L.push_back(hl[b] * t.len.mul + t.len.add);
        KX_HIP(hipMemcpy(tp.data.data() + (size_t)b * t.C * t.ld, t.p + (long)b * t.bs, (size_t)t.C * t.ld * 4,
                         hipMemcpyDeviceToHost));
    }
// ... 247 lines not shown
}

void Model::diag_enable(bool on) {
    sync();
    diag_on_ = on;
    diag_recs_.clear();
    diag_used_ = 0;
    if (on && !d_diag_) {
        diag_cap_ = 1024;
        d_diag_ = dev_alloc(3 * diag_cap_);
    }
    if (on) {
        KX_HIP(hipMemsetAsync(d_diag_, 0, 3 * diag_cap_ * sizeof(float), stream_));
        KX_HIP(hipStreamSynchronize(stream_));
    }
}

const std::vector<Model::DiagRec>& Model::diag_collect() {
    sync();
    std::vector<float> h(3 * diag_used_);
    if (diag_used_) KX_HIP(hipMemcpy(h.data(), d_diag_, h.size() * sizeof(float), hipMemcpyDeviceToHost));
    for (size_t i = 0; i < diag_recs_.size() && i < diag_used_; ++i) {
        diag_recs_[i].absmax = h[3 * i];
        diag_recs_[i].count = (double)h[3 * i + 2];
        diag_recs_[i].rms = diag_recs_[i].count > 0 ? std::sqrt((double)h[3 * i + 1] / diag_recs_[i].count) : 0.0;
    }
    return diag_recs_;
}

void Model::set_act_shift(const std::string& conv_name, int shift) {
    KX_REQUIRE(shift >= -24 && shift <= 24, "activation pre-scale: shift must be in -24..24");
    sync();
    auto it = convs_.find(conv_name);
    if (it != convs_.end()) {
        it->second.act_shift = shift;
        return;
    }
    const std::string suf = ".ih";
    if (conv_name.size() > suf.size() && conv_name.compare(conv_name.size() - suf.size(), suf.size(), suf) == 0) {
        auto il = lstms_.find(conv_name.substr(0, conv_name.size() - suf.size()));
        if (il != lstms_.end()) {
            il->second.ih.act_shift = shift;
            return;
        }
    }
    throw Error(4, "no such conv layer: " + conv_name);
}

int Model::get_act_shift(const std::string& conv_name) const {
    auto it = convs_.find(conv_name);
    if (it == convs_.end()) throw Error(4, "no such conv layer: " + conv_name);
    return it->second.act_shift;
}

void Model::profile_enable(bool on) {
    sync();
    prof_on_ = on;
    prof_recs_.clear();
    ev_used_ = 0;
    prof_flops_ = 0;
    prof_launches_ = 0;
    prof_stats_bytes_ = 0;
    prof_stats_launches_ = 0;
}

void Model::profile_aux(int64_t* stats_launches, double* stats_bytes) {
    if (!prof_on_) throw Error(4, "profiling is not enabled");
    *stats_launches = prof_stats_launches_;
    *stats_bytes = prof_stats_bytes_;
    prof_stats_launches_ = 0;
    prof_stats_bytes_ = 0;
}

void Model::profile_read(int64_t* launches, double* ms, double* flops) {
    if (!prof_on_) throw Error(4, "profiling is not enabled");
    sync();
    double total = 0;
    for (size_t i = 0; i + 1 < ev_used_; i += 2) {
        float t = 0;
        KX_HIP(hipEventElapsedTime(&t, ev_[i], ev_[i + 1]));
        total += t;
        if (i / 2 < prof_recs_.size()) prof_recs_[i / 2].ms = t;
    }
    prof_detail.swap(prof_recs_);
    prof_recs_.clear();
    *launches = prof_launches_;
    *ms = total;
    *flops = prof_flops_;
    ev_used_ = 0;
    prof_flops_ = 0;
    prof_launches_ = 0;
}

namespace {
struct DeviceGate {
    std::mutex mu;
    hipEvent_t last = nullptr;
    const void* owner = nullptr;
};
DeviceGate& device_gate(int dev) {
    static DeviceGate g[KX_MAX_DEVICES];
    if (dev < 0 || dev >= KX_MAX_DEVICES) throw Error(1, "device id outside 0.." + std::to_string(KX_MAX_DEVICES - 1));
    return g[dev];
}
bool device_turn_on() {
    static const bool on = !(getenv("KX_DEVICE_TURN") && atoi(getenv("KX_DEVICE_TURN")) == 0);
    return on;
}
}

struct Model::DeviceTurn {
    Model& m;
    DeviceGate& g;
    std::unique_lock<std::mutex> lk;
    const bool on;
    explicit DeviceTurn(Model& mm) : m(mm), g(device_gate(mm.device)), lk(g.mu, std::defer_lock), on(device_turn_on() && mm.n_parts_ == 1) {
        if (!on) return;
        lk.lock();
        if (g.last && g.owner != &m) KX_HIP(hipStreamWaitEvent(m.main_stream_, g.last, 0));
    }
    ~DeviceTurn() {
        if (!on) return;
        if (!g.last && hipEventCreateWithFlags(&g.last, hipEventDisableTiming) != hipSuccess) g.last = nullptr;
        if (g.last && hipEventRecord(g.last, m.main_stream_) == hipSuccess) g.owner = &m;
        else g.owner = nullptr;
    }
};

void Model::infer_device(const int64_t* d_ids, int64_t t_stride, const int32_t* lens_host, int B,
                         const float* d_styles, const float* speeds_host, int n_speed, uint64_t seed, uint32_t flags,
                         float* d_audio, int64_t audio_ld, int32_t* d_frames, int64_t* need_ld) {
    KX_REQUIRE(B >= 1 && B <= 4096, "infer: batch must be 1..4096 (empty input is an error)");
    KX_REQUIRE(d_ids && lens_host && d_styles && speeds_host, "infer: null argument");
    KX_REQUIRE(n_speed == 1 || n_speed == B, "infer: n_speed must be 1 or B");
    int Tmax = 0;
    for (int b = 0; b < B; ++b) {
        KX_REQUIRE(lens_host[b] >= 1 && lens_host[b] <= 512, "infer: token count must be 1..512");
        KX_REQUIRE((int64_t)lens_host[b] <= t_stride, "infer: lens[b] exceeds the row stride");
        if (lens_host[b] > Tmax) Tmax = lens_host[b];
    }
    for (int i = 0; i < n_speed; ++i) KX_REQUIRE(speeds_host[i] > 0.f, "infer: speed must be > 0");
    KX_HIP(hipSetDevice(device));
    CuScope cu_scope(cu_count_);
    using clk = std::chrono::steady_clock;
    const clk::time_point t_enter = clk::now();
    auto ms_since = [](clk::time_point t0) { return std::chrono::duration<double, std::milli>(clk::now() - t0).count(); };
    for (double& v : call_ms_) v = 0.0;
    DeviceTurn turn(*this);
    B_ = B;
    Tmax_ = Tmax;
    taps_on_ = (flags & 2u) != 0;
    taps_.clear();
    parts_.clear();
    p1_region_ = false;
    lane_ev_used_ = 0;
    prefix_keys_.clear();
    prefix_used_ = 0;
    n_lanes_ = prof_on_ ? 1 : (lanes_cfg_ ? lanes_cfg_ : (B <= 32 ? N_LANES : 1));
    hT_.assign(lens_host, lens_host + B);
    hF_.assign(B, 0);
    const int Tp = up4(Tmax);
    const int idx_ld = Tmax * 50;
    n_bs_ = 1104;
    const int noise_off = (flags & 1u) ? 1 : 0;
    if (lstm_exchange_bytes(B) > xchg_cap_) {
        KX_HIP(hipStreamSynchronize(stream_));
        for (auto*& p : d_xchg_) {
            if (p) KX_HIP(hipFree(p));
            p = nullptr;
            KX_HIP(hipMalloc((void**)&p, lstm_exchange_bytes(B)));
            KX_HIP(hipMemsetAsync(p, 0, lstm_exchange_bytes(B), stream_));
        }
        xchg_cap_ = lstm_exchange_bytes(B);
        xchg_epoch_[0] = xchg_epoch_[1] = 0;
    }

    float *emb, *h, *qkv, *ctx, *av, *ff, *dcat, *gxT, *gxT2, *xl, *logits, *te0, *te1, *t_en, *d_speeds;
    int *dur, *idx;
    auto planT = [&](Arena& A) {
        A.off = 0;
        dT_ = A.i(B);
        dF_ = A.i(B);
        d_bad_id_ = reinterpret_cast<unsigned*>(A.i(1));
        d_speeds = A.f(B);
        dur = A.i((size_t)B * 512);
        idx = A.i((size_t)B * idx_ld);
        gb_ = A.f((size_t)B * gb_total_);
        nmean_ = A.f((size_t)B * n_bs_);
        nscale_ = A.f((size_t)B * n_bs_);
        nshift_ = A.f((size_t)B * n_bs_);
        lanes_[0].nmean = nmean_;
        lanes_[0].nscale = nscale_;
        lanes_[0].nshift = nshift_;
        for (int i = 1; i < N_LANES; ++i) {
            lanes_[i].nmean = A.f((size_t)B * n_bs_);
            lanes_[i].nscale = A.f((size_t)B * n_bs_);
            lanes_[i].nshift = A.f((size_t)B * n_bs_);
        }
        const size_t bt = (size_t)B * Tp;
        emb = A.f(bt * 128);
        h = A.f(bt * 768);
        qkv = A.f(bt * 2304);
        ctx = A.f(bt * 768);
        av = A.f(bt * 768);
        ff = A.f(bt * 2048);
        dcat = A.f(bt * 640);
        gxT = A.f(bt * 2048);
        gxT2 = A.f(bt * 2048);
        xl = A.f(bt * 512);
        logits = A.f(bt * 50);
        te0 = A.f(bt * 512);
        te1 = A.f(bt * 512);
        t_en = A.f(bt * 512);
    };
    arenaT_.measure = true;
    planT(arenaT_);
    const size_t needT = arenaT_.off;
    arenaT_.measure = false;
    ensure_arena(arenaT_, needT);
    planT(arenaT_);

    KX_HIP(hipMemcpyAsync(dT_, lens_host, B * sizeof(int), hipMemcpyHostToDevice, stream_));
    KX_HIP(hipMemsetAsync(d_bad_id_, 0, sizeof(unsigned), stream_));
    KX_HIP(hipMemcpyAsync(d_speeds, speeds_host, n_speed * sizeof(float), hipMemcpyHostToDevice, stream_));
    const LenMap LT{dT_, 1, 0};
    auto TT = [&](float* p, int C) {
        T t;
        t.p = p; t.bs = (long)C * Tp; t.ld = Tp; t.C = C; t.len = LT; t.Lmax = Tmax;
        return t;
    };
    launch_style_fc(fc_dev_, (int)fc_host_.size(), d_styles, gb_, gb_total_, B, stream_);

    KX_HIP(hipEventRecord(ev_fork_, stream_));
    KX_HIP(hipStreamWaitEvent(stream2_, ev_fork_, 0));
    struct StreamSwap {
        hipStream_t &a, &b;
        StreamSwap(hipStream_t& x, hipStream_t& y) : a(x), b(y) { std::swap(a, b); }
        ~StreamSwap() { std::swap(a, b); }
    };
    T t_ten = TT(t_en, 512);
    {
    StreamSwap on_side(stream_, stream2_);
    T t_te0 = TT(te0, 512), t_te1 = TT(te1, 512);
    launch_embed(d_ids, t_stride, wt("text_encoder.embedding.weight"), 512, te0, t_te0.bs, Tp, dT_, B, Tmax, n_vocab_,
                 d_bad_id_, stream_);
    T* cur = &t_te0;
    T* nxt = &t_te1;
    for (int i = 0; i < 3; ++i) {
        ConvOpts o;
        o.pad = 2;
        conv(convs_.at("text_encoder.cnn." + std::to_string(i)), *cur, *nxt, o);
        const std::string ln = "text_encoder.cnn." + std::to_string(i) + ".1.";
        launch_layernorm_ch(nxt->p, nxt->p, nxt->bs, Tp, 512, LT, B, Tmax, 1e-5f, LN_AFFINE, wt(ln + "gamma"),
                            wt(ln + "beta"), 0, 0.2f, stream_);
        std::swap(cur, nxt);
    }
    tap("text_enc.cnn", *cur);
    lstm(lstms_.at("text_encoder.lstm"), *cur, t_ten, gxT2);
    tap("text_enc.out", t_ten);
    KX_HIP(hipEventRecord(ev_join_, stream_));
    }

    const std::string E = "bert.embeddings.";
    const std::string AL = "bert.encoder.albert_layer_groups.0.albert_layers.0.";
    T t_emb = TT(emb, 128), t_h = TT(h, 768), t_qkv = TT(qkv, 2304), t_ctx = TT(ctx, 768), t_a = TT(av, 768),
      t_f = TT(ff, 2048);
    launch_albert_embed(d_ids, t_stride, wt(E + "word_embeddings.weight"), wt(E + "token_type_embeddings.weight"),
                        wt(E + "position_embeddings.weight"), emb, t_emb.bs, Tp, dT_, B, Tmax, n_vocab_, d_bad_id_, stream_);
    launch_layernorm_ch(emb, emb, t_emb.bs, Tp, 128, LT, B, Tmax, 1e-12f, LN_AFFINE, wt(E + "LayerNorm.weight"),
                        wt(E + "LayerNorm.bias"), 0, 0.f, stream_);
    tap("bert.emb", t_emb);
    conv(convs_.at("bert.map"), t_emb, t_h, ConvOpts{});
    for (int l = 0; l < 12; ++l) {
        conv(convs_.at("bert.qkv"), t_h, t_qkv, ConvOpts{});
        launch_attention(qkv, t_qkv.bs, Tp, ctx, t_ctx.bs, Tp, dT_, B, Tmax, stream_);
        ConvOpts od;
        od.resid = &t_h;
        conv(convs_.at("bert.dense"), t_ctx, t_a, od);
        launch_layernorm_ch(av, av, t_a.bs, Tp, 768, LT, B, Tmax, 1e-12f, LN_AFFINE,
                            wt(AL + "attention.LayerNorm.weight"), wt(AL + "attention.LayerNorm.bias"), 0, 0.f, stream_);
        ConvOpts of;
        of.epi = EPI_GELU_NEW;
        conv(convs_.at("bert.ffn"), t_a, t_f, of);
        ConvOpts oo;
        oo.resid = &t_a;
        conv(convs_.at("bert.ffn_out"), t_f, t_h, oo);
        launch_layernorm_ch(h, h, t_h.bs, Tp, 768, LT, B, Tmax, 1e-12f, LN_AFFINE,
                            wt(AL + "full_layer_layer_norm.weight"), wt(AL + "full_layer_layer_norm.bias"), 0, 0.f,
                            stream_);
        if (l == 0) tap("bert.layer0", t_h);
    }
    tap("bert.out", t_h);

    T t_dcat = TT(dcat, 640);
    T t_d512 = t_dcat.rows(0, 512);
    conv(convs_.at("bert_encoder"), t_h, t_d512, ConvOpts{});
    tap("d_en", t_d512);
    launch_fill_style_rows(dcat, t_dcat.bs, Tp, 512, d_styles, 128, dT_, B, Tmax, stream_);
    for (int i = 0; i < 3; ++i) {
        lstm(lstms_.at("predictor.text_encoder.lstms." + std::to_string(2 * i)), t_dcat, t_d512, gxT);
        const float* g = gb_ + fc_off("dur_enc." + std::to_string(i));
        launch_layernorm_ch(dcat, dcat, t_dcat.bs, Tp, 512, LT, B, Tmax, 1e-5f, LN_ADA, g, g + 512, (int)gb_total_, 0.f,
                            stream_);
        tap(("dur_enc." + std::to_string(i)).c_str(), t_dcat);
    }
    T t_xl = TT(xl, 512), t_logits = TT(logits, 50);
    lstm(lstms_.at("predictor.lstm"), t_dcat, t_xl, gxT);
    tap("dur.lstm", t_xl);
    conv(convs_.at("duration_proj"), t_xl, t_logits, ConvOpts{});
    launch_duration(logits, t_logits.bs, Tp, d_speeds, n_speed, dT_, d_pinned_, n_pinned_, dur, dF_, idx, idx_ld, B,
                    stream_);
    KX_HIP(hipMemcpyAsync(hF_.data(), dF_, B * sizeof(int), hipMemcpyDeviceToHost, stream_));
    h_bad_id_ = 0;
    KX_HIP(hipMemcpyAsync(&h_bad_id_, d_bad_id_, sizeof(unsigned), hipMemcpyDeviceToHost, stream_));

    KX_HIP(hipStreamWaitEvent(stream_, ev_join_, 0));
    call_ms_[0] = ms_since(t_enter);
    KX_HIP(hipStreamSynchronize(stream_));
    call_ms_[1] = ms_since(t_enter);
    check_dev_err();
    if (h_bad_id_) {
        const unsigned w = h_bad_id_ - 1;
        throw Error(1, "infer: token id outside 0.." + std::to_string(n_vocab_ - 1) + " (utterance " + std::to_string(w >> 16) +
                           ", position " + std::to_string(w & 0xffffu) + ")");
    }
    int Fmax = 0;
    for (int b = 0; b < B; ++b) Fmax = hF_[b] > Fmax ? hF_[b] : Fmax;
    Fmax_ = Fmax;
    if (need_ld) *need_ld = (int64_t)600 * Fmax;
    if (d_frames) KX_HIP(hipMemcpyAsync(d_frames, dF_, B * sizeof(int), hipMemcpyDeviceToDevice, stream_));
    if (audio_ld < (int64_t)600 * Fmax || !d_audio)
        throw Error(1, "infer: audio buffer too small, need ld >= " + std::to_string((long long)600 * Fmax));

    const int F1p = up4(Fmax), F2p = up4(2 * Fmax), F20p = up4(20 * Fmax), F120p = up4(120 * Fmax + 1);
    const LenMap LF1{dF_, 1, 0}, LF2{dF_, 2, 0}, LF20{dF_, 20, 0}, LF120{dF_, 120, 0}, LF121{dF_, 120, 1};
    auto mk = [&](Arena& A, int C, int ld, LenMap len, int Lmax) {
        T t;
        t.p = A.f((size_t)B * C * ld);
        t.bs = (long)C * ld; t.ld = ld; t.C = C; t.len = len; t.Lmax = Lmax;
        return t;
    };
    auto back = [&](Arena& A) {
        A.off = 0;
        stats_arena_ = &A;
        img_arena_ = &A;
        auto F1 = [&](int C) { return mk(A, C, F1p, LF1, Fmax); };
        auto F2 = [&](int C) { return mk(A, C, F2p, LF2, 2 * Fmax); };
        auto F20 = [&](int C) { return mk(A, C, F20p, LF20, 20 * Fmax); };
        auto F121 = [&](int C) { return mk(A, C, F120p, LF121, 120 * Fmax + 1); };
        T en = F1(640);
        if (!dry_) launch_gather_cols(dcat, t_dcat.bs, Tp, en.p, en.bs, en.ld, 640, idx, idx_ld, dF_, B, Fmax, stream_);
        float* gxF = A.f((size_t)B * Fmax * 2048);
        T xsh = F1(512);
        lstm(lstms_.at("predictor.shared"), en, xsh, gxF);
        tap("pred.shared", xsh);
        T curves = F2(2);
        stats(xsh, "predictor.F0.0.norm1");
        hipEvent_t ev_n = nullptr;
        for (int br = 1; br >= 0; --br) {
            const std::string P = std::string("predictor.") + (br == 0 ? "F0" : "N");
            LaneScope on_lane(*this, br);
            T y0 = F1(512);
            adain_resblk(P + ".0", xsh, y0, false, A.f((size_t)B * 512 * F1p), nullptr, nullptr);
            T y1 = F2(256);
            float* wa = A.f((size_t)B * 256 * F2p);
            float* wb = A.f((size_t)B * 256 * F2p);
            float* wc = A.f((size_t)B * 512 * F2p);
            adain_resblk(P + ".1", y0, y1, true, wa, wb, wc);
            T y2 = F2(256);
            adain_resblk(P + ".2", y1, y2, false, A.f((size_t)B * 256 * F2p), nullptr, nullptr);
            conv(convs_.at(P + "_proj"), y2, curves.rows(br, 1), ConvOpts{});
            if (br == 1) ev_n = record_here();
        }
        wait_here(ev_n);
        tap("pred.F0", curves.rows(0, 1));
        tap("pred.N", curves.rows(1, 1));
        const std::string G = "decoder.generator.";
        T ns[2];
        hipEvent_t ev_ns[2] = {nullptr, nullptr};
        size_t part_n[2];
        p1_region_ = true;
        {
            LaneScope on_lane(*this, 3);
            const long hs_ld = (long)600 * Fmax;
            float* har_src = A.f((size_t)B * hs_ld);
            float* phase = A.f((size_t)B * 9 * 2 * Fmax);
            if (!dry_)
                launch_source(curves.p, curves.bs, dF_, B, Fmax, wt(G + "m_source.l_linear.weight"),
                              wt(G + "m_source.l_linear.bias"), seed, utt_base, d_utt_seeds_, noise_off, phase, har_src, hs_ld, stream_);
            if (taps_on_ && !dry_) {
                T hs;
                hs.p = har_src; hs.bs = hs_ld; hs.ld = (int)hs_ld; hs.C = 1; hs.len = LenMap{dF_, 600, 0}; hs.Lmax = 600 * Fmax;
                tap("gen.har_source", hs);
            }
            T har = F121(22);
            if (!dry_) launch_stft(har_src, hs_ld, har.p, har.bs, har.ld, dF_, B, Fmax, stft_variant, stream_);
            tap("gen.har", har);
            for (int st = 0; st < 2; ++st) {
                const int ch = st == 0 ? 256 : 128;
                auto S = [&](int C) { return st == 0 ? F20(C) : F121(C); };
                ns[st] = S(ch);
                T t1 = S(ch);
                part_n[st] = (size_t)B * ch * ((st == 0 ? 20 * Fmax : 120 * Fmax + 1) / 64 + 4);
                float2* part_t1 = static_cast<float2*>(A.alloc(part_n[st] * sizeof(float2)));
                float2* part_xj = static_cast<float2*>(A.alloc(part_n[st] * sizeof(float2)));
                {
                    ConvOpts o;
                    if (st == 0) { o.stride = 6; o.pad = 3; }
                    o.stat_part = part_xj;
                    conv(convs_.at(G + "noise_convs." + std::to_string(st)), har, ns[st], o);
                }
                adain_resblock1(G + "noise_res." + std::to_string(st), st == 0 ? 7 : 11, ns[st], ns[st], t1, ns[st], 0, 1.f,
                                part_t1, part_xj);
                tap(("gen.x_source." + std::to_string(st)).c_str(), ns[st]);
                ev_ns[st] = record_here();
            }
        }
        T xcat0 = F1(514);
        if (!dry_)
            launch_gather_cols(t_en, t_ten.bs, Tp, xcat0.p, xcat0.bs, xcat0.ld, 512, idx, idx_ld, dF_, B, Fmax, stream_);
        {
            ConvOpts o;
            o.stride = 2;
            o.pad = 1;
            conv(convs_.at("decoder.F0_conv"), curves.rows(0, 1), xcat0.rows(512, 1), o);
            conv(convs_.at("decoder.N_conv"), curves.rows(1, 1), xcat0.rows(513, 1), o);
        }
        T catA = F1(1090), catB = F1(1090);
        float* wa = A.f((size_t)B * 1024 * F1p);
        float* wb = A.f((size_t)B * 1024 * F1p);
        adain_resblk("decoder.encode", xcat0, catA.rows(0, 1024), false, wa, wb, nullptr);
        tap("dec.encode", catA.rows(0, 1024));
        conv(convs_.at("decoder.asr_res"), xcat0.rows(0, 512), catA.rows(1024, 64), ConvOpts{});
        if (!dry_) {
            launch_copy_rows(xcat0.rows(512, 2).p, xcat0.bs, xcat0.ld, catA.rows(1088, 2).p, catA.bs, catA.ld, 2, LF1, B,
                             Fmax, stream_);
            launch_copy_rows(catA.rows(1024, 66).p, catA.bs, catA.ld, catB.rows(1024, 66).p, catB.bs, catB.ld, 66, LF1,
                             B, Fmax, stream_);
        }
        T* ci = &catA;
        T* co = &catB;
        for (int i = 0; i < 3; ++i) {
// ... 399 lines not shown
```

kokorox_amd/hip_koko.py:

```python
from __future__ import annotations

import ctypes as C
import os
from typing import List, Optional, Sequence

import numpy as np

_HERE = os.path.dirname(os.path.abspath(__file__))
LIB_PATH = os.path.join(_HERE, "lib", "libkokorox_hip.so")

PACK_F32_MONO, PACK_F32_STEREO, PACK_PCM16_MONO = 0, 1, 2
KX_OK, KX_ERR_INVALID, KX_ERR_IO, KX_ERR_DEVICE, KX_ERR_STATE = 0, 1, 2, 3, 4
KX_FLAG_NOISE_OFF = 1
KX_FLAG_TAPS = 2
STYLE_DIM = 256
SAMPLES_PER_FRAME = 600

_lib = None


class KokoroxHipError(RuntimeError):
    def __init__(self, code: int, msg: str):
        super().__init__(f"kokorox_hip error {code}: {msg}")
        self.code = code


def load_library(path: Optional[str] = None) -> C.CDLL:
    global _lib
    if _lib is not None and path is None:
        return _lib
    import sys
    p = path or os.environ.get("KX_LIB") or LIB_PATH
    import sys
    if "torch" not in sys.modules and os.environ.get("KX_NO_TORCH_PRELOAD") != "1":
        try:
            import torch
        except Exception:
            pass
    if not os.path.exists(p) and p == LIB_PATH and os.environ.get("KX_NO_AUTOBUILD") != "1":
        try:
            from . import build as _build
            _build.build_library(verbose=True)
        except Exception as e:
            print(f"kokorox_amd: building libkokorox_hip.so failed: {e}", file=sys.stderr)
    if not os.path.exists(p):
        raise FileNotFoundError(
            f"{p} is missing: build it with `python -m kokorox_amd.build` (hipcc, gfx950). "
            "The HIP path has no CPU fallback.")
    lib = C.CDLL(p)
    vp, i32, i64, u32, u64, f32 = C.c_void_p, C.c_int, C.c_int64, C.c_uint32, C.c_uint64, C.c_float
    cp, sz = C.c_char_p, C.c_size_t
    sig = {
        "kx_version": (cp, []),
        "kx_init": (i32, [i32, cp, sz]),
        "kx_create": (vp, [cp, i32, cp, sz]),
        "kx_import_onnx": (i32, [cp, cp, cp, sz]),
        "kx_warmup": (i32, [vp, i32, i32, i32]),
        "kx_arena_bytes": (i32, [vp, C.POINTER(i64)]),
        "kx_call_times": (i32, [vp, C.POINTER(C.c_double)]),
        "kx_model_status": (i32, [vp, C.POINTER(i64)]),
        "kx_model_info": (i32, [vp, C.POINTER(i64)]),
        "kx_dispatcher_health": (i32, [vp, vp, i32, C.POINTER(i64), C.POINTER(i64)]),
        "kx_create_from_device_blob": (vp, [vp, sz, i32, cp, sz]),
        "kx_destroy": (None, [vp]),
        "kx_last_error": (cp, [vp]),
        "kx_last_error_copy": (i32, [vp, cp, sz]),
        "kx_create_replicas": (i32, [cp, vp, i32, vp, cp, sz]),
        "kx_replicas_times": (i32, [C.POINTER(C.c_double)]),
        "kx_create_partition": (vp, [cp, i32, i32, i32, cp, sz]),
        "kx_infer": (i32, [vp, vp, i64, vp, i32, vp, vp, i32, u64, u32, C.POINTER(C.POINTER(f32)), vp]),
        "kx_free_audio": (None, [C.POINTER(f32)]),
        "kx_infer_device": (i32, [vp, vp, i64, vp, i32, vp, vp, i32, u64, u32, vp, i64, vp, C.POINTER(i64)]),
        "kx_sync": (i32, [vp]),
        "kx_set_pinned_durations": (i32, [vp, vp, i32]),
        "kx_set_utterance_base": (i32, [vp, u64]),
        "kx_set_lanes": (i32, [vp, i32]),
        "kx_set_conv_mode": (i32, [vp, i32]),
        "kx_get_conv_mode": (i32, [vp]),
        "kx_set_stft_variant": (i32, [vp, i32]),
        "kx_get_stft_variant": (i32, [vp]),
        "kx_profile_enable": (i32, [vp, i32]),
        "kx_profile_read": (i32, [vp, C.POINTER(i64), C.POINTER(C.c_double), C.POINTER(C.c_double)]),
        "kx_profile_detail": (i32, [vp, vp, i64, C.POINTER(i64)]),
        "kx_profile_aux": (i32, [vp, C.POINTER(i64), C.POINTER(C.c_double)]),
        "kx_diag_enable": (i32, [vp, i32]),
        "kx_diag_count": (i32, [vp, C.POINTER(i64)]),
        "kx_diag_get": (i32, [vp, i64, cp, sz, vp]),
        "kx_set_act_prescale": (i32, [vp, cp, i32]),
        "kx_set_voice_table": (i32, [vp, vp, i32]),
        "kx_infer_voices": (i32, [vp, vp, i64, vp, i32, vp, vp, i32, vp, i32, u64, u32, i32, C.POINTER(vp), vp, vp]),
        "kx_infer_packed": (i32, [vp, vp, i64, vp, i32, vp, vp, i32, u64, u32, i32, C.POINTER(vp), vp, vp]),
        "kx_free_packed": (None, [vp]),
        "kx_dispatcher_create": (vp, [vp, i32, i32, i32, cp, sz]),
        "kx_dispatcher_create_warm": (vp, [vp, i32, i32, i32, i32, i32, cp, sz]),
        "kx_dispatcher_submit": (i32, [vp, vp, i32, vp, f32, u64, C.POINTER(C.POINTER(f32)), C.POINTER(i64), cp, sz]),
        "kx_dispatcher_submit_ex": (i32, [vp, vp, i32, vp, vp, vp, i32, f32, u64, i32, C.POINTER(vp), C.POINTER(i64),
                                          C.POINTER(i64), cp, sz]),
        "kx_dispatcher_stats": (i32, [vp, C.POINTER(i64), C.POINTER(i64), C.POINTER(i64)]),
        "kx_dispatcher_model_batches": (i32, [vp, vp, i32]),
        "kx_dispatcher_failures": (i32, [vp, C.POINTER(i64), C.POINTER(i64)]),
        "kx_dispatcher_destroy": (None, [vp]),
        "kx_debug_tap": (i32, [vp, cp, i32, vp, i64, C.POINTER(C.c_int32), C.POINTER(C.c_int32)]),
    }
    for name, (res, args) in sig.items():
        fn = getattr(lib, name)
        fn.restype = res
        fn.argtypes = args
    if path is None:
        _lib = lib
    return lib


TEST_LIB_PATH = os.path.join(os.path.dirname(LIB_PATH), "libkokorox_hip_test.so")
_test_lib = None


def load_test_library() -> C.CDLL:
    global _test_lib
    if _test_lib is not None:
        return _test_lib
    load_library()
    p = os.environ.get("KX_TEST_LIB") or TEST_LIB_PATH
    if not os.path.exists(p):
        raise FileNotFoundError(f"{p} is missing: build it with `python -m kokorox_amd.build` (hipcc, gfx950)")
    lib = C.CDLL(p)
    vp, i32, i64, u32, u64, f32 = C.c_void_p, C.c_int, C.c_int64, C.c_uint32, C.c_uint64, C.c_float
    cp, sz = C.c_char_p, C.c_size_t
    sig = {
        "kx_test_conv1d": (i32, [i32, vp, i32, i32, i32, vp, vp, i32, i32, i32, i32, i32, i32, i32, f32, vp, vp, vp,
                                 i32, i32, cp, sz]),
        "kx_test_conv1d_full": (i32, [i32, vp, i32, i32, i32, vp, i32, vp, vp, i32, i32, i32, i32, i32, f32, vp, vp, vp, i32, f32,
                                      f32, vp, vp, i32, cp, sz]),
        "kx_test_conv_transpose": (i32, [i32, vp, i32, i32, i32, vp, vp, i32, i32, i32, f32, vp, i32, vp, i32, cp, sz]),
        "kx_test_lstm": (i32, [i32, vp, i32, i32, i32] + [vp] * 9 + [cp, sz]),
        "kx_test_source": (i32, [i32, vp, i32, i32, vp, f32, u64, u64, i32, vp, cp, sz]),
        "kx_test_attention": (i32, [i32, vp, vp, i32, i32, vp, cp, sz]),
        "kx_test_lstm_fault": (i32, [i32]),
        "kx_test_conv1d_epilogue": (i32, [i32, vp, i32, i32, i32, vp, vp, i32, i32, i32, i32, vp, i32, f32, f32, vp, vp,
                                          i32, cp, sz]),
        "kx_test_lstm_parts": (i32, [i32]),
        "kx_test_conv_plan": (i32, [vp, i32, vp, i32, cp, sz]),
    }
    for name, (res, args) in sig.items():
        fn = getattr(lib, name)
        fn.restype = res
        fn.argtypes = args
    _test_lib = lib
    return lib


TEST_ABI_SYMBOLS = ["kx_test_conv1d", "kx_test_lstm", "kx_test_source", "kx_test_attention", "kx_test_conv1d_epilogue", "kx_test_conv1d_full",
                    "kx_test_conv_transpose", "kx_test_lstm_fault", "kx_test_lstm_parts", "kx_test_conv_plan"]

ABI_SYMBOLS = [
    "kx_version", "kx_init", "kx_create", "kx_import_onnx", "kx_create_from_device_blob", "kx_create_replicas", "kx_replicas_times", "kx_create_partition", "kx_destroy",
    "kx_last_error", "kx_last_error_copy", "kx_infer",
    "kx_free_audio", "kx_infer_device", "kx_sync", "kx_set_pinned_durations", "kx_warmup", "kx_arena_bytes", "kx_call_times", "kx_model_status", "kx_model_info", "kx_dispatcher_health", "kx_set_utterance_base", "kx_set_lanes",
    "kx_set_conv_mode", "kx_get_conv_mode", "kx_set_stft_variant", "kx_get_stft_variant",
    "kx_profile_enable", "kx_profile_read", "kx_profile_detail", "kx_profile_aux", "kx_diag_enable", "kx_diag_count", "kx_diag_get", "kx_set_act_prescale", "kx_set_voice_table", "kx_infer_voices",
    "kx_infer_packed", "kx_free_packed", "kx_dispatcher_create", "kx_dispatcher_create_warm", "kx_dispatcher_submit", "kx_dispatcher_submit_ex", "kx_dispatcher_model_batches",
    "kx_dispatcher_stats", "kx_dispatcher_failures", "kx_dispatcher_destroy", "kx_debug_tap",
]


def _ptr(a: Optional[np.ndarray]):
    return None if a is None else a.ctypes.data_as(C.c_void_p)


def _f32(a) -> Optional[np.ndarray]:
    return None if a is None else np.ascontiguousarray(a, dtype=np.float32)


class HipKoko:

    def __init__(self, model_path: str, device: int = 0, _handle=None):
        self._lib = load_library()
        self.device = device
        if _handle is not None:
            self._h = _handle
            return
        err = C.create_string_buffer(512)
        h = self._lib.kx_create(os.fsencode(model_path), device, err, len(err))
        if not h:
            raise RuntimeError(f"Failed to create Kokoro TTS model: {err.value.decode()}")
        self._h = h

    @classmethod
    def new(cls, model_path: str, device: int = 0) -> "HipKoko":
        return cls(model_path, device)

    @classmethod
    def from_device_blob(cls, data_ptr: int, n_bytes: int, device: int = 0) -> "HipKoko":
        lib = load_library()
        err = C.create_string_buffer(512)
        h = lib.kx_create_from_device_blob(C.c_void_p(data_ptr), n_bytes, device, err, len(err))
        if not h:
            raise RuntimeError(f"Failed to create Kokoro TTS model: {err.value.decode()}")
        return cls("", device, _handle=h)

    @classmethod
    def replicas(cls, model_path: str, devices: Sequence[int]) -> List["HipKoko"]:
        lib = load_library()
        dev = np.ascontiguousarray(devices, dtype=np.int32)
        if dev.ndim != 1 or dev.shape[0] < 1:
            raise ValueError("replicas: at least one device id")
        out = (C.c_void_p * dev.shape[0])()
        err = C.create_string_buffer(512)
        rc = lib.kx_create_replicas(os.fsencode(model_path), _ptr(dev), dev.shape[0], out, err, len(err))
        if rc != 0:
            raise RuntimeError(f"Failed to create Kokoro TTS model: {err.value.decode()}")
        return [cls("", int(d), _handle=out[i]) for i, d in enumerate(dev)]

    @staticmethod
    def replicas_times():
        out = (C.c_double * 3)()
        load_library().kx_replicas_times(out)
        return list(out)

    @classmethod
    def partition(cls, model_path: str, device: int, part: int, n_parts: int) -> "HipKoko":
        lib = load_library()
        err = C.create_string_buffer(512)
        h = lib.kx_create_partition(os.fsencode(model_path), device, part, n_parts, err, len(err))
        if not h:
            raise RuntimeError(f"Failed to create Kokoro TTS model: {err.value.decode()}")
        return cls("", device, _handle=h)

    def last_error(self) -> str:
        buf = C.create_string_buffer(512)
        self._lib.kx_last_error_copy(self._h, buf, len(buf))
        return buf.value.decode()

    def infer(self, tokens: Sequence[Sequence[int]], styles: Sequence[Sequence[float]], speed: float,
              seed: int = 0, flags: int = 0):
        if len(tokens) == 0 or len(tokens[0]) == 0:
            raise ValueError("infer: empty token list")
        if len(styles) != len(tokens):
            raise ValueError("infer: one style row per utterance is required")
        outs = self.infer_batch(tokens, styles, [float(speed)], seed=seed, flags=flags)
        return outs[0] if len(outs) == 1 else outs

    def infer_batch(self, tokens, styles, speeds, seed: int = 0, flags: int = 0) -> List[np.ndarray]:
        B = len(tokens)
        lens = np.array([len(t) for t in tokens], dtype=np.int32)
        stride = int(lens.max()) if B else 0
        ids = np.zeros((B, max(stride, 1)), dtype=np.int64)
        for b, t in enumerate(tokens):
            ids[b, : len(t)] = np.asarray(t, dtype=np.int64)
        st = _f32(np.asarray(styles, dtype=np.float32).reshape(B, -1))
        if B and st.shape[1] != STYLE_DIM:
            raise ValueError(f"infer: style rows must have {STYLE_DIM} floats")
        sp = _f32(np.asarray(speeds, dtype=np.float32).reshape(-1))
        out = C.POINTER(C.c_float)()
        out_lens = np.zeros(max(B, 1), dtype=np.int64)
        rc = self._lib.kx_infer(self._h, _ptr(ids), ids.shape[1], _ptr(lens), B, _ptr(st), _ptr(sp), sp.shape[0],
                                seed, flags, C.byref(out), _ptr(out_lens))
        self._check(rc)
        try:
            total = int(out_lens[:B].sum())
            flat = np.ctypeslib.as_array(out, shape=(max(total, 1),))[:total].copy()
        finally:
            self._lib.kx_free_audio(out)
        res, o = [], 0
        for b in range(B):
            res.append(flat[o: o + int(out_lens[b])])
            o += int(out_lens[b])
        return res

    def set_voice_table(self, table: np.ndarray):
        t = _f32(np.asarray(table, dtype=np.float32).reshape(-1, 511, 256))
        self._check(self._lib.kx_set_voice_table(self._h, _ptr(t), t.shape[0]))

    def _unpack(self, out, nbytes, nsamp, B, fmt):
        total = int(nbytes[:B].sum())
        raw = C.string_at(out, total) if total else b""
        self._lib.kx_free_packed(out)
        res, o = [], 0
        dt = np.int16 if fmt == PACK_PCM16_MONO else np.float32
        for b in range(B):
            a = np.frombuffer(raw, dtype=dt, count=int(nbytes[b]) // np.dtype(dt).itemsize, offset=o).copy()
            res.append(a.reshape(-1, 2) if fmt == PACK_F32_STEREO else a)
            o += int(nbytes[b])
        return res

    def _ids_lens(self, tokens):
        B = len(tokens)
        lens = np.array([len(t) for t in tokens], dtype=np.int32)
        ids = np.zeros((B, max(int(lens.max()), 1)), dtype=np.int64)
        for b, t in enumerate(tokens):
            ids[b, : len(t)] = np.asarray(t, dtype=np.int64)
        return ids, lens

    def infer_voices(self, tokens, voice_ids, weights, speeds=(1.0,), seed: int = 0, flags: int = 0,
                     fmt: int = 0) -> List[np.ndarray]:
        ids, lens = self._ids_lens(tokens)
        B = len(tokens)
        v = np.ascontiguousarray(np.asarray(voice_ids, dtype=np.int32).reshape(B, -1))
        w = _f32(np.asarray(weights, dtype=np.float32).reshape(B, -1))
        sp = _f32(np.asarray(speeds, dtype=np.float32).reshape(-1))
        out = C.c_void_p()
        nbytes, nsamp = np.zeros(B, np.int64), np.zeros(B, np.int64)
        self._check(self._lib.kx_infer_voices(self._h, _ptr(ids), ids.shape[1], _ptr(lens), B, _ptr(v), _ptr(w),
                                              v.shape[1], _ptr(sp), sp.shape[0], seed, flags, fmt, C.byref(out),
                                              _ptr(nbytes), _ptr(nsamp)))
        return self._unpack(out, nbytes, nsamp, B, fmt)
# ... 115 lines not shown

    def tap(self, name: str, b: int = 0) -> np.ndarray:
        c, l = C.c_int32(0), C.c_int32(0)
        self._check(self._lib.kx_debug_tap(self._h, name.encode(), b, None, 0, C.byref(c), C.byref(l)))
        out = np.empty((c.value, l.value), dtype=np.float32)
        self._check(self._lib.kx_debug_tap(self._h, name.encode(), b, _ptr(out), out.size, C.byref(c), C.byref(l)))
        return out

    def close(self):
        if getattr(self, "_h", None):
            self._lib.kx_destroy(self._h)
            self._h = None

    def __del__(self):
        try:
            self.close()
        except Exception:
            pass

    def _check(self, rc: int):
        if rc != 0:
            raise KokoroxHipError(rc, self.last_error())


class Dispatcher:

    def __init__(self, models: Sequence[HipKoko], max_batch: int = 64, max_wait_us: int = 2000, warm: Optional[Sequence[int]] = None):
        self._lib = load_library()
        self._models = list(models)
        arr = (C.c_void_p * len(self._models))(*[m._h for m in self._models])
        err = C.create_string_buffer(256)
        if warm:
            self._d = self._lib.kx_dispatcher_create_warm(arr, len(self._models), max_batch, max_wait_us, int(warm[0]), int(warm[1]), err, len(err))
        else:
            self._d = self._lib.kx_dispatcher_create(arr, len(self._models), max_batch, max_wait_us, err, len(err))
        if not self._d:
            raise RuntimeError(f"dispatcher: {err.value.decode()}")

    def submit(self, ids: Sequence[int], style: Sequence[float], speed: float = 1.0, seed: int = 0) -> np.ndarray:
        a = np.ascontiguousarray(ids, dtype=np.int64)
        st = _f32(np.asarray(style, dtype=np.float32).reshape(-1))
        if st.shape[0] != STYLE_DIM:
            raise ValueError(f"style row must have {STYLE_DIM} floats")
        out = C.POINTER(C.c_float)()
        n = C.c_int64(0)
        err = C.create_string_buffer(256)
        rc = self._lib.kx_dispatcher_submit(self._d, _ptr(a), a.shape[0], _ptr(st), float(speed), seed, C.byref(out),
                                            C.byref(n), err, len(err))
        if rc != 0:
            raise KokoroxHipError(rc, err.value.decode())
        try:
            return np.ctypeslib.as_array(out, shape=(max(n.value, 1),))[: n.value].copy()
        finally:
            self._lib.kx_free_audio(out)

    def submit_ex(self, ids: Sequence[int], style: Optional[Sequence[float]] = None,
                  voices: Optional[Sequence] = None, speed: float = 1.0, seed: int = 0, fmt: int = 0) -> np.ndarray:
        a = np.ascontiguousarray(ids, dtype=np.int64)
        st = vid = w = None
        n_mix = 0
        if style is not None:
            st = _f32(np.asarray(style, dtype=np.float32).reshape(-1))
            if st.shape[0] != STYLE_DIM:
                raise ValueError(f"style row must have {STYLE_DIM} floats")
        elif isinstance(voices, (int, np.integer)):
            vid, n_mix = np.array([voices], dtype=np.int32), 1
        else:
            vid = np.array([v for v, _ in voices], dtype=np.int32)
            w = np.array([x for _, x in voices], dtype=np.float32)
            n_mix = len(vid)
        out, nb, ns = C.c_void_p(), C.c_int64(0), C.c_int64(0)
        err = C.create_string_buffer(256)
        rc = self._lib.kx_dispatcher_submit_ex(self._d, _ptr(a), a.shape[0], _ptr(st), _ptr(vid), _ptr(w), n_mix,
                                               float(speed), seed, fmt, C.byref(out), C.byref(nb), C.byref(ns), err, len(err))
        if rc != 0:
            raise KokoroxHipError(rc, err.value.decode())
        try:
            raw = C.string_at(out, nb.value)
        finally:
            self._lib.kx_free_audio(C.cast(out, C.POINTER(C.c_float)))
        if fmt == 2:
            return np.frombuffer(raw, dtype=np.int16).copy()
        arr = np.frombuffer(raw, dtype=np.float32).copy()
        return arr.reshape(-1, 2) if fmt == 1 else arr

    def stats(self):
        a, b, c = C.c_int64(0), C.c_int64(0), C.c_int64(0)
        self._lib.kx_dispatcher_stats(self._d, C.byref(a), C.byref(b), C.byref(c))
        per = (C.c_int64 * len(self._models))()
        self._lib.kx_dispatcher_model_batches(self._d, per, len(self._models))
        rp, rt = C.c_int64(0), C.c_int64(0)
        self._lib.kx_dispatcher_failures(self._d, C.byref(rp), C.byref(rt))
        hl = (C.c_int32 * len(self._models))()
        mf, rq = C.c_int64(0), C.c_int64(0)
        self._lib.kx_dispatcher_health(self._d, hl, len(self._models), C.byref(mf), C.byref(rq))
        return {"requests": a.value, "batches": b.value, "max_batch": c.value, "batches_per_model": list(per),
                "replayed_requests": rp.value, "retried_batches": rt.value, "healthy": [int(v) for v in hl],
                "failed_models": mf.value, "requeued_requests": rq.value}

    def close(self):
        if getattr(self, "_d", None):
            self._lib.kx_dispatcher_destroy(self._d)
            self._d = None

    def __del__(self):
        try:
            self.close()
        except Exception:
            pass


def import_onnx(onnx_path: str, out_path: str) -> str:
    lib = load_library()
    err = C.create_string_buffer(2048)
    rc = lib.kx_import_onnx(os.fsencode(onnx_path), os.fsencode(out_path), err, len(err))
    if rc != KX_OK:
        raise KokoroxHipError(rc, err.value.decode(errors="replace"))
    return out_path


def _err_call(fn, *args):
    err = C.create_string_buffer(512)
    rc = fn(*args, err, len(err))
    if rc != 0:
        raise KokoroxHipError(rc, err.value.decode())


CONV_F32, CONV_F16X3, CONV_F16F8 = 0, 1, 6
STFT_ONNX, STFT_TORCH = 0, 1


def conv1d(x, w, bias=None, stride=1, pad=0, dil=1, transposed=False, act=0, slope=0.0, alpha=None, norm=None,
           device=0, mode=None, pre=False):
    lib = load_test_library()
    if mode is None:
        mode = CONV_F32 if os.environ.get("KOKOROX_CONV", "") == "f32" else CONV_F16X3
    x, w = _f32(x), _f32(w)
    B, Cin, L = x.shape
    k = w.shape[2]
    if transposed:
        Cout = w.shape[1]
        Lout = (L - 1) * stride - 2 * pad + k
    else:
        Cout = w.shape[0]
        Lout = (L + 2 * pad - dil * (k - 1) - 1) // stride + 1
    y = np.zeros((B, Cout, Lout), dtype=np.float32)
    bias, alpha, norm = _f32(bias), _f32(alpha), _f32(norm)
    _err_call(lib.kx_test_conv1d, device, _ptr(x), B, Cin, L, _ptr(w), _ptr(bias), Cout, k, stride, pad, dil,
              1 if transposed else 0, act, float(slope), _ptr(alpha), _ptr(norm), _ptr(y), Lout, mode | (0x100 if pre else 0))
    return y


CONV_LAUNCH_FIELDS = ("mode", "prec1", "f8", "BM", "rows", "n_chunks16", "K", "dil", "stride", "pad", "act", "in_up2", "store", "accum",
                      "epi", "norm", "stats", "image", "merge_T", "x_bs", "x_ld", "B", "cols", "cus", "force")
CONV_PLAN_FIELDS = ("form", "bm", "act", "kt", "wm", "wn", "vt", "pf", "p1", "bf", "bn", "cols", "merged", "pre", "stat_cols",
                    "stat_tiles", "flat_bn")
CONV_FORMS = ("F32", "LDS", "DAG", "DAGN", "DA", "DA_W2", "DA_S16", "DA_F8", "DA_PRE", "DAPN")


def conv_plan(**launch):
    lib = load_test_library()
    unknown = set(launch) - set(CONV_LAUNCH_FIELDS)
    assert not unknown, unknown
    src = np.array([int(launch.get(f, 0)) for f in CONV_LAUNCH_FIELDS], dtype=np.int64)
    out = np.zeros(len(CONV_PLAN_FIELDS), dtype=np.int64)
    _err_call(lib.kx_test_conv_plan, _ptr(src), len(src), _ptr(out), len(out))
    plan = dict(zip(CONV_PLAN_FIELDS, (int(v) for v in out)))
    plan["form"] = CONV_FORMS[plan["form"]]
    return plan


def conv_transpose(x, w, bias=None, stride=6, act=1, slope=0.1, resid=None, up_off=0, mode=1, pre=False, device=0):
    lib = load_test_library()
    x, w = _f32(x), _f32(w)
    B, Cin, L = x.shape
    Cout, k = w.shape[1], w.shape[2]
    assert k == 2 * stride
    pad = (k - stride) // 2
    Lout = (L - 1) * stride - 2 * pad + k
    y = np.zeros((B, Cout, Lout + (1 if up_off else 0)), dtype=np.float32)
    _err_call(lib.kx_test_conv_transpose, device, _ptr(x), B, Cin, L, _ptr(w), _ptr(_f32(bias)), Cout, stride, act, float(slope),
              _ptr(_f32(resid)), 1 if up_off else 0, _ptr(y), mode | (0x100 if pre else 0))
    return y


def conv1d_epilogue(x, w, bias=None, pad=0, dil=1, resid=None, y_init=None, out_mul=1.0, out_div=1.0, want_stats=False,
                    mode=1, device=0):
    lib = load_test_library()
    x, w = _f32(x), _f32(w)
    B, Cin, L = x.shape
    Cout, _, k = w.shape
    Lout = L + 2 * pad - dil * (k - 1)
    y = np.zeros((B, Cout, Lout), dtype=np.float32) if y_init is None else _f32(y_init).copy()
    st = np.zeros((B, Cout, 2), dtype=np.float32) if want_stats else None
    _err_call(lib.kx_test_conv1d_epilogue, device, _ptr(x), B, Cin, L, _ptr(w), _ptr(_f32(bias)), Cout, k, pad, dil,
              _ptr(_f32(resid)), 0 if y_init is None else 1, float(out_mul), float(out_div), _ptr(y), _ptr(st), mode)
    return (y, st) if want_stats else y


def conv1d_full(x, w, bias=None, pad=0, dil=1, act=0, slope=0.0, alpha=None, norm=None, resid=None, y_init=None,
                out_mul=1.0, out_div=1.0, want_stats=False, lens=None, pad_ld=False, flat=False, mode=1, device=0, pre=False):
    lib = load_test_library()
    x, w = _f32(x), _f32(w)
    B, Cin, L = x.shape
    Cout, _, k = w.shape
    Lout = L + 2 * pad - dil * (k - 1)
    y = np.zeros((B, Cout, Lout), dtype=np.float32) if y_init is None else _f32(y_init).copy()
    st = np.zeros((B, Cout, 2), dtype=np.float32) if want_stats else None
    ln = None if lens is None else np.ascontiguousarray(lens, dtype=np.int32)
    _err_call(lib.kx_test_conv1d_full, device, _ptr(x), B, Cin, L, _ptr(ln), (1 if pad_ld else 0) | (2 if flat else 0), _ptr(w), _ptr(_f32(bias)),
              Cout, k, pad, dil, act, float(slope), _ptr(_f32(alpha)), _ptr(_f32(norm)), _ptr(_f32(resid)),
              0 if y_init is None else 1, float(out_mul), float(out_div), _ptr(y), _ptr(st), mode | (0x100 if pre else 0))
    return (y, st) if want_stats else y


def lstm(x, params, device=0):
    lib = load_test_library()
    x = _f32(x)
    B, L, n_in = x.shape
    ps = [_f32(p) for p in params]
    y = np.zeros((B, L, 512), dtype=np.float32)
    _err_call(lib.kx_test_lstm, device, _ptr(x), B, L, n_in, *[_ptr(p) for p in ps], _ptr(y))
    return y


def attention(qkv, lens, device=0):
    lib = load_test_library()
    qkv = _f32(qkv)
    B, C, T = qkv.shape
    assert C == 2304
    lens = np.ascontiguousarray(np.asarray(lens, dtype=np.int32))
    ctx = np.zeros((B, 768, T), dtype=np.float32)
    _err_call(lib.kx_test_attention, device, _ptr(qkv), _ptr(lens), B, T, _ptr(ctx))
    return ctx


def harmonic_source(f0, lin_w, lin_b, seed=0, utt_base=0, noise_off=False, device=0):
    lib = load_test_library()
    f0 = _f32(f0)
    B, F2 = f0.shape
    lin_w = _f32(np.asarray(lin_w).reshape(-1))
    out = np.zeros((B, 300 * F2), dtype=np.float32)
    _err_call(lib.kx_test_source, device, _ptr(f0), B, F2, _ptr(lin_w), float(lin_b), seed, utt_base,
              1 if noise_off else 0, _ptr(out))
    return out
```

Before: 6875 x realtime.

## Feed BERT GEMMs pre-split f16 input images produced by layernorm, attention and GEMM epilogues

Adds a DAGI k=1 GEMM kernel that reads a pre-split hi/lo f16 input image instead of splitting f32 activations inside the GEMM. Layernorm, attention and the FFN GEMM epilogue now also write that split image, and when every consumer reads the image the f32 output is skipped. The BERT loop wires these images between layers, aiming to cut repeated split work and f32 traffic in the 12-layer encoder. It adds image buffers, a new planner route and more complex epilogues.

```diff
diff --git a/kokorox_amd/build.py b/kokorox_amd/build.py
--- a/kokorox_amd/build.py
+++ b/kokorox_amd/build.py
@@ -10,7 +10,7 @@
 LIB_PATH = os.path.join(LIB_DIR, "libkokorox_hip.so")
 TEST_LIB_PATH = os.path.join(LIB_DIR, "libkokorox_hip_test.so")
 TEST_SOURCES = ["test_hooks.hip"]
-SOURCES = ["conv_plan.hip", "conv_mfma.hip", "conv_f16x3.hip", "conv_f16x3_da.hip", "conv_f16x3_da_p1.hip", "conv_f16x3_da_w2.hip", "conv_f16x3_da_s16.hip", "conv_f16x3_da_f8.hip", "conv_f16x3_da_pre.hip", "conv_f16x3_pre.hip", "conv_f16x3_dapn.hip", "conv_f16x3_dag.hip", "kernels_misc.hip", "model.hip", "api.hip", "dispatcher.hip", "onnx_import.cpp"]
+SOURCES = ["conv_plan.hip", "conv_mfma.hip", "conv_f16x3.hip", "conv_f16x3_da.hip", "conv_f16x3_da_p1.hip", "conv_f16x3_da_w2.hip", "conv_f16x3_da_s16.hip", "conv_f16x3_da_f8.hip", "conv_f16x3_da_pre.hip", "conv_f16x3_pre.hip", "conv_f16x3_dapn.hip", "conv_f16x3_dag.hip", "conv_f16x3_dagi.hip", "kernels_misc.hip", "model.hip", "api.hip", "dispatcher.hip", "onnx_import.cpp"]
 HEADERS = ["kx_common.h", "kx_error.h", "conv_epilogue.h", "conv_f16x3_common.h"]
 _PUB = os.path.join("..", "..", "include", "kokorox_hip.h")
 _PUB_TEST = os.path.join("..", "..", "include", "kokorox_hip_test.h")
diff --git a/kokorox_amd/csrc/conv_f16x3.hip b/kokorox_amd/csrc/conv_f16x3.hip
--- a/kokorox_amd/csrc/conv_f16x3.hip
+++ b/kokorox_amd/csrc/conv_f16x3.hip
@@ -399,7 +399,7 @@
         return;
     }
     KX_REQUIRE(a.n_chunks16 == (a.Cin + CK16 - 1) / CK16 && a.w16 != nullptr, "conv1d f16x3: weights not packed");
-    KX_REQUIRE(a.epi != EPI_GELU_NEW || p.vt > 1 || p.form == FORM_DAG || p.form == FORM_DAGN,
+    KX_REQUIRE(a.epi != EPI_GELU_NEW || p.vt > 1 || p.form == FORM_DAG || p.form == FORM_DAGN || p.form == FORM_DAGI,
                "conv1d f16x3: gelu epilogue exists only for k=1 GEMMs with >= 48 input channels");
     KX_REQUIRE(p.merged == (a.merge_T > 0), "conv1d f16x3: merged columns do not match the plan");
     if (p.cols <= 0) return;
@@ -407,6 +407,7 @@
         case FORM_LDS: launch_lds(p, a, B, s); return;
         case FORM_DAG:
         case FORM_DAGN: launch_conv1d_f16x3_dag(p, a, B, s); return;
+        case FORM_DAGI: launch_conv1d_f16x3_dagi(p, a, B, s); return;
         case FORM_DAPN: launch_conv1d_f16x3_dapn(a, B, p.cols, s); return;
         case FORM_DA_PRE: launch_conv16_da_pre(p, a, B, s); return;
         case FORM_DA_S16: launch_conv16_da_s16(p, a, B, s); return;
diff --git a/kokorox_amd/csrc/conv_f16x3_dagi.hip b/kokorox_amd/csrc/conv_f16x3_dagi.hip
--- /dev/null
+++ b/kokorox_amd/csrc/conv_f16x3_dagi.hip
@@ -0,0 +1,277 @@
+#include "conv_f16x3_common.h"
+#include <type_traits>
+
+namespace kx {
+
+template <int I, int N, class F>
+__device__ __forceinline__ void static_for_i(F&& f) {
+    if constexpr (I < N) {
+        f(std::integral_constant<int, I>{});
+        static_for_i<I + 1, N>(f);
+    }
+}
+
+__device__ __forceinline__ void dagi_store_image(const ConvArgs& a, f32x16 (&acc)[1][4], float acc_scale, int b, int row0, int col0,
+                                                 int r, int h, int ncols) {
+    const bool gelu = a.epi == EPI_GELU_NEW;
+    const bool merged = a.merge_T > 0;
+    const int rmax = a.Cout - 1;
+    const int brow = row0 + r + 32 * h;
+    const float bias_lane = a.bias ? a.bias[brow < rmax ? brow : rmax] : 0.f;
+#pragma unroll
+    for (int nt = 0; nt < 4; ++nt) {
+        const int col = col0 + nt * 32 + r;
+        const bool cok = col < ncols;
+        const int cc = cok ? col : ncols - 1;
+        int bb = b, tt = cc;
+        if (merged) {
+            bb = cc / a.merge_T;
+            tt = cc - bb * a.merge_T;
+        }
+        float* yb = a.y + (long)bb * a.y_bs + tt;
+        const float* rb = a.resid ? a.resid + (long)bb * a.r_bs + tt : nullptr;
+        unsigned char* ib = static_cast<unsigned char*>(a.y16) + (long)bb * a.y16_bs + (long)tt * 16 + 8 * h;
+#pragma unroll
+        for (int q = 0; q < 4; ++q) {
+            float v[4];
+#pragma unroll
+            for (int j = 0; j < 4; ++j) {
+                const int e = 4 * q + j, c = j + 8 * q;
+                const float b0 = __builtin_bit_cast(float, __builtin_amdgcn_readlane(__builtin_bit_cast(int, bias_lane), c));
+                const float b1 = __builtin_bit_cast(float, __builtin_amdgcn_readlane(__builtin_bit_cast(int, bias_lane), c + 4));
+                const int row = row0 + c + 4 * h;
+                const int rl = row < rmax ? row : rmax;
+                float x = __builtin_fmaf(acc[0][nt][e], acc_scale, h ? b1 : b0);
+                if (rb) x += rb[(long)rl * a.r_ld];
+                x *= a.out_mul;
+                if (gelu) x = gelu_new_f(x);
+                if (cok && row <= rmax && !a.y16_only) yb[(long)row * a.y_ld] = x;
+                v[j] = x * a.y16_prescale;
+            }
+            uint2 hi, lo;
+            split_pair(v[0], v[1], hi.x, lo.x);
+            split_pair(v[2], v[3], hi.y, lo.y);
+            const int rowq = row0 + 8 * q;
+            if (cok && rowq <= rmax) {
+                const long slot = (long)((rowq >> 4) * 4 + (q & 1)) * a.y16_ld;
+                *reinterpret_cast<uint2*>(ib + slot * 16) = hi;
+                *reinterpret_cast<uint2*>(ib + (slot + 2L * a.y16_ld) * 16) = lo;
+            }
+        }
+    }
+}
+
+template <bool IMG_OUT>
+__global__ __launch_bounds__(256, 3) void conv1d_f16x3_dagi_kernel(const ConvArgs a) {
+    constexpr int BM = 128, BN = 128, NT = 4, VT = 3;
+    constexpr int XWp = BN;
+    constexpr int XIMG = 4 * XWp;
+    constexpr int XBUF = VT * XIMG;
+    constexpr int tap_units = 4 * BM;
+    extern __shared__ __attribute__((aligned(16))) unsigned char smem16[];
+    uint4* Xs = reinterpret_cast<uint4*>(smem16);
+
+    const int tid = threadIdx.x;
+    const int lane = tid & 63;
+    const int wave = __builtin_amdgcn_readfirstlane(tid >> 6);
+    const int r = lane & 31, h = lane >> 5;
+    const int b = blockIdx.z;
+    int tile_x = blockIdx.x, ct = blockIdx.y;
+    {
+        const int nx = gridDim.x, ny = gridDim.y, N = nx * ny;
+        const int l = blockIdx.x + nx * blockIdx.y;
+        int lp = l;
+        if (a.xcd_swizzle && N >= 16) {
+            const int off = (int)(((long)N * blockIdx.z) & 7);
+            const int cls = (l + off) & 7;
+            int start = 0;
+            for (int c = 0; c < cls; ++c) {
+                const int first = (c - off) & 7;
+                start += first < N ? (N - first + 7) >> 3 : 0;
+            }
+            lp = start + (l >> 3);
+        }
+        if (a.xcd_swizzle) {
+            tile_x = lp / ny;
+            ct = lp - tile_x * ny;
+        }
+    }
+    const int t0 = tile_x * BN;
+    const bool merged = a.merge_T > 0;
+    const int Lin = merged ? a.merge_B * a.merge_T : a.in_len.lens[b] * a.in_len.mul + a.in_len.add;
+    const int Lout = merged ? Lin : a.out_len.lens[b] * a.out_len.mul + a.out_len.add;
+    const int ncols = Lout;
+    if (t0 >= ncols) return;
+
+    const int n_chunks = a.n_chunks16;
+    const int n_super = (n_chunks + VT - 1) / VT;
+
+    f32x16 acc[1][NT];
+#pragma unroll
+    for (int j = 0; j < NT; ++j)
+#pragma unroll
+        for (int e = 0; e < 16; ++e) acc[0][j][e] = 0.f;
+
+    using u32x4 = __attribute__((ext_vector_type(4))) unsigned;
+    const int u = tid & 127, g = wave >> 1;
+    const uint4* ibase;
+    bool pok;
+    {
+        const int p = t0 + u;
+        const int pc = p < Lin ? p : Lin - 1;
+        long off;
+        if (merged) {
+            const int bb = pc / a.merge_T, tt = pc - bb * a.merge_T;
+            pok = p < Lin && tt < a.in_len.lens[bb];
+            off = (long)bb * (a.x16_bs >> 4) + tt;
+        } else {
+            pok = p < Lin;
+            off = (long)b * (a.x16_bs >> 4) + pc;
+        }
+        ibase = static_cast<const uint4*>(a.x16) + off + (long)g * a.x16_ld;
+    }
+    constexpr int img_ops = 2 * VT;
+    u32x4 ximg[img_ops];
+    auto load_img = [&](int sc) __attribute__((always_inline)) {
+#pragma unroll
+        for (int vt = 0; vt < VT; ++vt) {
+            const int c = sc * VT + vt;
+            const uint4* p = ibase + (long)(c < n_chunks ? c : n_chunks - 1) * 4 * a.x16_ld;
+            asm volatile("global_load_dwordx4 %0, %1, off" : "=v"(ximg[2 * vt]) : "v"(p) : "memory");
+            asm volatile("global_load_dwordx4 %0, %1, off" : "=v"(ximg[2 * vt + 1]) : "v"(p + 2L * a.x16_ld) : "memory");
+        }
+    };
+    auto put_img = [&](const int k, uint4* Xb, int sc) __attribute__((always_inline)) {
+        const int vt = k >> 1, pl = k & 1;
+        const bool ok = pok && sc * VT + vt < n_chunks;
+        const u32x4 v = ximg[k];
+        Xb[vt * XIMG + (pl * 2 + g) * XWp + u] = make_uint4(ok ? v[0] : 0u, ok ? v[1] : 0u, ok ? v[2] : 0u, ok ? v[3] : 0u);
+    };
+    auto hand_img = [&]() __attribute__((always_inline)) {
+        __builtin_amdgcn_sched_barrier(0);
+        asm volatile("" : "+v"(ximg[0]), "+v"(ximg[1]), "+v"(ximg[2]), "+v"(ximg[3]), "+v"(ximg[4]), "+v"(ximg[5]));
+    };
+
+    const uint4* wlane = reinterpret_cast<const uint4*>(a.w16) + (long)ct * n_chunks * tap_units + h * BM + wave * 32 + r;
+    auto load_A = [&](int s, u32x4& a_hi, u32x4& a_lo) __attribute__((always_inline)) {
+        const int sc = s < n_chunks ? s : n_chunks - 1;
+        const uint4* p = wlane + (long)sc * tap_units;
+        asm volatile("global_load_dwordx4 %0, %1, off" : "=v"(a_hi) : "v"(p) : "memory");
+        asm volatile("global_load_dwordx4 %0, %1, off" : "=v"(a_lo) : "v"(p + 2 * BM) : "memory");
+    };
+    auto wait_A = [&](int age, u32x4& a_hi, u32x4& a_lo) __attribute__((always_inline)) {
+        if (age >= 10) asm volatile("s_waitcnt vmcnt(10)" ::: "memory");
+        else if (age >= 8) asm volatile("s_waitcnt vmcnt(8)" ::: "memory");
+        else if (age >= 6) asm volatile("s_waitcnt vmcnt(6)" ::: "memory");
+        else if (age >= 4) asm volatile("s_waitcnt vmcnt(4)" ::: "memory");
+        else if (age >= 2) asm volatile("s_waitcnt vmcnt(2)" ::: "memory");
+        else asm volatile("s_waitcnt vmcnt(0)" ::: "memory");
+        __builtin_amdgcn_sched_barrier(0);
+        asm volatile("" : "+v"(a_hi), "+v"(a_lo));
+    };
+
+    u32x4 ahs[3], als[3];
+    load_A(0, ahs[0], als[0]);
+    load_A(1, ahs[1], als[1]);
+    load_A(2, ahs[2], als[2]);
+    load_img(0);
+    asm volatile("s_waitcnt vmcnt(0)" ::: "memory");
+    hand_img();
+#pragma unroll
+    for (int k = 0; k < img_ops; ++k) put_img(k, Xs, 0);
+    __syncthreads();
+    int ages[3] = {0, 0, 0};
+    if (n_super > 1) {
+        load_img(1);
+        ages[0] = ages[1] = ages[2] = img_ops;
+    }
+
+    int cur = 0;
+    half8 fh[3], fl[3];
+    auto load_tile = [&](int vt, int n, half8& fhx, half8& flx) __attribute__((always_inline)) {
+        const uint4* xt = Xs + cur * XBUF + vt * XIMG + h * XWp + r + n * 32;
+        fhx = *reinterpret_cast<const half8*>(xt);
+        flx = *reinterpret_cast<const half8*>(xt + 2 * XWp);
+    };
+    load_tile(0, 0, fh[0], fl[0]);
+    load_tile(0, 1, fh[1], fl[1]);
+    constexpr int TILES = NT * VT;
+    constexpr int PUT0 = 8;
+    for (int sc = 0; sc < n_super; ++sc) {
+        const bool more = sc + 1 < n_super;
+        static_for_i<0, TILES>([&](auto ic) __attribute__((always_inline)) {
+            constexpr int i = decltype(ic)::value;
+            constexpr int t = i / NT, n = i % NT, sl = t;
+            constexpr int e = i % 3, ip = i + 2, e2 = ip % 3;
+            if constexpr (n == 0) wait_A(ages[sl], ahs[sl], als[sl]);
+            const half8 ah = __builtin_bit_cast(half8, ahs[sl]), al = __builtin_bit_cast(half8, als[sl]);
+            if constexpr (ip < TILES) load_tile(ip / NT, ip % NT, fh[e2], fl[e2]);
+            __builtin_amdgcn_sched_barrier(0);
+            acc[0][n] = __builtin_amdgcn_mfma_f32_32x32x16_f16(al, fh[e], acc[0][n], 0, 0, 0);
+            acc[0][n] = __builtin_amdgcn_mfma_f32_32x32x16_f16(ah, fl[e], acc[0][n], 0, 0, 0);
+            acc[0][n] = __builtin_amdgcn_mfma_f32_32x32x16_f16(ah, fh[e], acc[0][n], 0, 0, 0);
+            if constexpr (i >= PUT0) {
+                if (more) {
+                    if constexpr (i == PUT0) {
+                        __builtin_amdgcn_sched_barrier(0);
+                        asm volatile("s_waitcnt vmcnt(4)" ::: "memory");
+                        hand_img();
+                    }
+                    constexpr int k0 = i == PUT0 ? 0 : (i == PUT0 + 1 ? 2 : i - PUT0 + 2), k1 = i <= PUT0 + 1 ? k0 + 2 : k0 + 1;
+#pragma unroll
+                    for (int k = k0; k < k1; ++k) put_img(k, Xs + (cur ^ 1) * XBUF, sc + 1);
+                }
+            }
+            __builtin_amdgcn_sched_barrier(0);
+            if constexpr (n == NT - 1) {
+                if (more) {
+                    load_A((sc + 1) * VT + t, ahs[sl], als[sl]);
+#pragma unroll
+                    for (int o = 0; o < 3; ++o) ages[o] = o == sl ? 0 : ages[o] + 2;
+                }
+            }
+        });
+        if (more) {
+            asm volatile("s_waitcnt lgkmcnt(0)\n\ts_barrier" ::: "memory");
+            cur ^= 1;
+            if (sc + 2 < n_super) {
+                load_img(sc + 2);
+#pragma unroll
+                for (int o = 0; o < 3; ++o) ages[o] += img_ops;
+            }
+            load_tile(0, 0, fh[0], fl[0]);
+            load_tile(0, 1, fh[1], fl[1]);
+        }
+    }
+
+    asm volatile("s_waitcnt vmcnt(0)" ::: "memory");
+    if constexpr (IMG_OUT)
+        dagi_store_image(a, acc, a.w_unscale, b, ct * BM + wave * 32, t0, r, h, ncols);
+    else
+        conv_store_tile<1, NT, EPI_ROWS, true>(a, acc, a.w_unscale, b, ct * BM + wave * 32, t0, r, h, ncols, Lout, tile_x, nullptr);
+}
+
+void launch_conv1d_f16x3_dagi(const ConvPlan& p, const ConvArgs& a, int B, hipStream_t s) {
+    KX_REQUIRE(a.K == 1 && a.stride == 1 && !a.stat_part && !a.in_up2 && a.n_chunks16 >= 3 && a.act == ACT_NONE && a.nmean == nullptr &&
+                   a.store != ST_UPSCATTER && a.pad == 0,
+               "conv1d f16x3 dag image: launch not eligible");
+    KX_REQUIRE(a.n_chunks16 == (a.Cin + CK16 - 1) / CK16 && a.w16 != nullptr, "conv1d f16x3 dag image: weights not packed");
+    KX_REQUIRE(a.x16 != nullptr && a.x16_bs % 16 == 0 && (size_t)a.x16_bs >= conv16_pre_image_bytes(a.Cin, a.x16_ld),
+               "conv1d f16x3 dag image: no input image");
+    if (p.cols <= 0) return;
+    constexpr size_t lds = 16 * (size_t)2 * 3 * 4 * 128;
+    dim3 grid((p.cols + 127) / 128, (a.Cout + 127) / 128, a.merge_T > 0 ? 1 : B);
+    KX_REQUIRE(grid.x > 0 && grid.y > 0 && grid.y < 65536 && B > 0 && B < 65536, "conv1d f16x3 dag image: bad grid");
+    if (a.y16) {
+        KX_REQUIRE(a.store == ST_NORMAL && !a.accum && a.Cout % 16 == 0 && a.y16_bs % 16 == 0 &&
+                       (size_t)a.y16_bs >= conv16_pre_image_bytes(a.Cout, a.y16_ld),
+                   "conv1d f16x3 dag image: the output image needs a plain store of whole chunks");
+        hipLaunchKernelGGL(conv1d_f16x3_dagi_kernel<true>, grid, dim3(256), lds, s, a);
+    } else {
+        KX_REQUIRE(!a.y16_only, "conv1d f16x3 dag image: nothing to store");
+        hipLaunchKernelGGL(conv1d_f16x3_dagi_kernel<false>, grid, dim3(256), lds, s, a);
+    }
+    KX_HIP(hipGetLastError());
+}
+
+}
diff --git a/kokorox_amd/csrc/conv_plan.hip b/kokorox_amd/csrc/conv_plan.hip
--- a/kokorox_amd/csrc/conv_plan.hip
+++ b/kokorox_amd/csrc/conv_plan.hip
@@ -62,7 +62,8 @@
         if (route != FORCE_LDS && !c.norm && c.store != ST_UPSCATTER) {
             const long wgs = tiles * (p.merged ? 1 : c.B);
             const bool narrow_ok = (c.x_bs * c.B + 16L * c.x_ld) * 4 < (1L << 31);
-            p.form = narrow_ok && 2 * wgs <= c.cus ? FORM_DAGN : FORM_DAG;
+            p.form = narrow_ok && 2 * wgs <= c.cus && !(c.force & FORCE_DAG_WIDE) ? FORM_DAGN : FORM_DAG;
+            if (p.form == FORM_DAG && c.x_image && c.act == ACT_NONE && (c.mode == CONV_F16X3 || c.mode == CONV_F16F8)) p.form = FORM_DAGI;
             p.bn = p.form == FORM_DAGN ? 32 : 128;
             return p;
         }
diff --git a/kokorox_amd/csrc/kernels_misc.hip b/kokorox_amd/csrc/kernels_misc.hip
--- a/kokorox_amd/csrc/kernels_misc.hip
+++ b/kokorox_amd/csrc/kernels_misc.hip
@@ -2,6 +2,7 @@
 
 #include <atomic>
 
+#include "conv_f16x3_common.h"
 #include "kx_common.h"
 
 namespace kx {
@@ -65,11 +66,14 @@
     KX_HIP(hipGetLastError());
 }
 
-template <int CPT>
+constexpr int LN_IMG_PITCH = 18;
+template <int CPT, bool IMG>
 __global__ __launch_bounds__(1024) void layernorm_ch_kernel(const float* x, float* y, long bs, int ld, int C,
                                                             LenMap len, float eps, int mode, const float* g,
-                                                            const float* be, int g_bs, float leaky) {
+                                                            const float* be, int g_bs, float leaky, uint4* img, long img_bs_u4,
+                                                            float img_prescale) {
     __shared__ float red[2][16][16];
+    extern __shared__ __attribute__((aligned(16))) float ln_tile[];
     const int tx = threadIdx.x & 15, cg = threadIdx.x >> 4, wave = threadIdx.x >> 6;
     const bool wave_lead = (threadIdx.x & 63) < 16;
     const int b = blockIdx.y, t = blockIdx.x * 16 + tx;
@@ -107,12 +111,12 @@
 #pragma unroll
     for (int k = 0; k < 16; ++k) qt += red[1][k][tx];
     const float rstd = 1.0f / sqrtf(qt / (float)C + eps);
-    if (!ok) return;
+    if (!IMG && !ok) return;
     float* yb = y + b * bs + t;
 #pragma unroll
     for (int i = 0; i < CPT; ++i) {
         const int c = cg + 64 * i;
-        if (c >= C) continue;
+        if (c >= C || !ok) continue;
         float o = (v[i] - mean) * rstd;
         if (mode == LN_AFFINE)
             o = o * g[c] + be[c];
@@ -120,24 +124,57 @@
             o = (1.0f + g[(long)b * g_bs + c]) * o + be[(long)b * g_bs + c];
         if (leaky != 0.f) o = o > 0.f ? o : o * leaky;
         yb[(long)c * ld] = o;
-    }
+        if (IMG) ln_tile[c * LN_IMG_PITCH + tx] = o;
+    }
+    if (IMG) {
+        __syncthreads();
+        const int t0 = blockIdx.x * 16;
+        uint4* ib = img + b * img_bs_u4;
+        for (int idx = threadIdx.x; idx < (C >> 3) * 16; idx += 1024) {
+            const int col = idx & 15, oc = idx >> 4;
+            if (t0 + col >= L) continue;
+            unsigned hp[4], lp[4];
+#pragma unroll
+            for (int c2 = 0; c2 < 4; ++c2) {
+                const float* src = ln_tile + (oc * 8 + 2 * c2) * LN_IMG_PITCH + col;
+                split_pair(src[0] * img_prescale, src[LN_IMG_PITCH] * img_prescale, hp[c2], lp[c2]);
+            }
+            uint4* slot = ib + (long)((oc >> 1) * 4 + (oc & 1)) * ld + t0 + col;
+            slot[0] = make_uint4(hp[0], hp[1], hp[2], hp[3]);
+            slot[2L * ld] = make_uint4(lp[0], lp[1], lp[2], lp[3]);
+        }
+    }
+}
+template <int CPT>
+static void launch_ln_inst(dim3 grid, const float* x, float* y, long bs, int ld, int C, LenMap len, float eps, int mode, const float* g,
+                           const float* be, int g_bs, float leaky, hipStream_t s, void* img, long img_bs, float img_prescale) {
+    if (img) {
+        const size_t lds = (size_t)C * LN_IMG_PITCH * sizeof(float);
+        hipLaunchKernelGGL((layernorm_ch_kernel<CPT, true>), grid, dim3(1024), lds, s, x, y, bs, ld, C, len, eps, mode, g, be, g_bs, leaky,
+                           static_cast<uint4*>(img), img_bs / 16, img_prescale);
+    } else
+        hipLaunchKernelGGL((layernorm_ch_kernel<CPT, false>), grid, dim3(1024), 0, s, x, y, bs, ld, C, len, eps, mode, g, be, g_bs, leaky,
+                           (uint4*)nullptr, 0L, 1.f);
 }
 void launch_layernorm_ch(const float* x, float* y, long bs, int ld, int C, LenMap len, int B, int Lmax, float eps,
-                         int mode, const float* g, const float* be, int g_bs, float leaky, hipStream_t s) {
+                         int mode, const float* g, const float* be, int g_bs, float leaky, hipStream_t s, void* img, long img_bs,
+                         float img_prescale) {
     if (Lmax <= 0) return;
     KX_REQUIRE(C <= 768, "layernorm: at most 768 channels");
-    const dim3 grid((Lmax + 15) / 16, B), block(1024);
+    KX_REQUIRE(!img || (C % 16 == 0 && img_bs % 16 == 0 && (size_t)img_bs >= conv16_pre_image_bytes(C, ld)), "layernorm: bad image geometry");
+    const dim3 grid((Lmax + 15) / 16, B);
     if (C <= 128)
-        hipLaunchKernelGGL(layernorm_ch_kernel<2>, grid, block, 0, s, x, y, bs, ld, C, len, eps, mode, g, be, g_bs, leaky);
+        launch_ln_inst<2>(grid, x, y, bs, ld, C, len, eps, mode, g, be, g_bs, leaky, s, img, img_bs, img_prescale);
     else if (C <= 512)
-        hipLaunchKernelGGL(layernorm_ch_kernel<8>, grid, block, 0, s, x, y, bs, ld, C, len, eps, mode, g, be, g_bs, leaky);
+        launch_ln_inst<8>(grid, x, y, bs, ld, C, len, eps, mode, g, be, g_bs, leaky, s, img, img_bs, img_prescale);
     else
-        hipLaunchKernelGGL(layernorm_ch_kernel<12>, grid, block, 0, s, x, y, bs, ld, C, len, eps, mode, g, be, g_bs, leaky);
+        launch_ln_inst<12>(grid, x, y, bs, ld, C, len, eps, mode, g, be, g_bs, leaky, s, img, img_bs, img_prescale);
     KX_HIP(hipGetLastError());
 }
 
 __global__ __launch_bounds__(256) void attention_mfma_kernel(const float* qkv, long bs, int ld, float* ctx, long cbs,
-                                                             int cld, const int* lens) {
+                                                             int cld, const int* lens, unsigned char* img, long img_bs,
+                                                             float img_prescale, int img_only) {
     using f32x16 = __attribute__((ext_vector_type(16))) float;
     const int b = blockIdx.x, hd = blockIdx.y;
     const int lane = threadIdx.x & 63, wave = threadIdx.x >> 6;
@@ -215,19 +252,42 @@
         float* cb = ctx + b * cbs + (long)(hd * 64) * cld + q0 + i;
 #pragma unroll
         for (int e = 0; e < 16; ++e) {
-            const int d = (e & 3) + 8 * (e >> 2) + 4 * hh;
-            cb[(long)d * cld] = o0[e] * inv;
-            cb[(long)(32 + d) * cld] = o1[e] * inv;
+            o0[e] *= inv;
+            o1[e] *= inv;
+        }
+        if (!img_only) {
+#pragma unroll
+            for (int e = 0; e < 16; ++e) {
+                const int d = (e & 3) + 8 * (e >> 2) + 4 * hh;
+                cb[(long)d * cld] = o0[e];
+                cb[(long)(32 + d) * cld] = o1[e];
+            }
+        }
+        if (img) {
+            unsigned char* ib = img + b * img_bs + (long)(q0 + i) * 16 + 8 * hh;
+#pragma unroll
+            for (int q = 0; q < 8; ++q) {
+                const int e0 = 4 * (q & 3);
+                const float v0 = (q < 4 ? o0[e0] : o1[e0]) * img_prescale, v1 = (q < 4 ? o0[e0 + 1] : o1[e0 + 1]) * img_prescale;
+                const float v2 = (q < 4 ? o0[e0 + 2] : o1[e0 + 2]) * img_prescale, v3 = (q < 4 ? o0[e0 + 3] : o1[e0 + 3]) * img_prescale;
+                uint2 hi, lo;
+                split_pair(v0, v1, hi.x, lo.x);
+                split_pair(v2, v3, hi.y, lo.y);
+                const long slot = (long)((hd * 4 + (q >> 1)) * 4 + (q & 1)) * cld;
+                *reinterpret_cast<uint2*>(ib + slot * 16) = hi;
+                *reinterpret_cast<uint2*>(ib + (slot + 2L * cld) * 16) = lo;
+            }
         }
     }
 }
 
 void launch_attention(const float* qkv, long bs, int ld, float* ctx, long cbs, int cld, const int* lens, int B,
-                      int Tmax, hipStream_t s) {
+                      int Tmax, hipStream_t s, void* img, long img_bs, float img_prescale, int img_only) {
     KX_REQUIRE(Tmax <= 512, "attention: T > 512");
     KX_REQUIRE(ld % 32 == 0 && ld >= ((Tmax + 31) & ~31), "attention: rows must be padded to a multiple of 32 columns");
+    KX_REQUIRE(img ? (img_bs % 16 == 0 && (size_t)img_bs >= conv16_pre_image_bytes(768, cld)) : !img_only, "attention: bad image geometry");
     hipLaunchKernelGGL(attention_mfma_kernel, dim3(B, 12, (Tmax + 127) / 128), dim3(256), 0, s, qkv, bs, ld, ctx, cbs,
-                       cld, lens);
+                       cld, lens, static_cast<unsigned char*>(img), img_bs, img_prescale, img_only);
     KX_HIP(hipGetLastError());
 }
 
diff --git a/kokorox_amd/csrc/kx_common.h b/kokorox_amd/csrc/kx_common.h
--- a/kokorox_amd/csrc/kx_common.h
+++ b/kokorox_amd/csrc/kx_common.h
@@ -115,6 +115,11 @@
     const void* x16;
     long x16_bs;
     int x16_ld;
+    void* y16;
+    long y16_bs;
+    int y16_ld;
+    float y16_prescale;
+    int y16_only;
 };
 
 enum ConvMode { CONV_F32 = 0, CONV_F16X3 = 1, CONV_F16X3_LDS = 2, CONV_F16X3_DA = 3, CONV_F16 = 4, CONV_BF16 = 5, CONV_F16F8 = 6 };
@@ -129,8 +134,9 @@
     FORM_DA_F8,
     FORM_DA_PRE,
     FORM_DAPN,
-};
-enum ConvForce { FORCE_LDS = 1, FORCE_DA = 2, FORCE_DA_4X1 = 4, FORCE_NO_S16 = 8 };
+    FORM_DAGI,
+};
+enum ConvForce { FORCE_LDS = 1, FORCE_DA = 2, FORCE_DA_4X1 = 4, FORCE_NO_S16 = 8, FORCE_DAG_WIDE = 16 };
 
 struct ConvLaunch {
     int mode;
@@ -146,6 +152,7 @@
     int B, cols;
     int cus;
     int force;
+    int x_image;
 };
 struct ConvPlan {
     int form;
@@ -188,6 +195,7 @@
 void launch_conv16_da_pre(const ConvPlan& p, const ConvArgs& a, int B, hipStream_t s);
 void launch_conv1d_f16x3_dapn(const ConvArgs& a, int B, int max_cols, hipStream_t s);
 void launch_conv1d_f16x3_dag(const ConvPlan& p, const ConvArgs& a, int B, hipStream_t s);
+void launch_conv1d_f16x3_dagi(const ConvPlan& p, const ConvArgs& a, int B, hipStream_t s);
 size_t packed_conv16_halves(int rows, int Cin, int K, int BM);
 float device_absmax(const float* p, long n, hipStream_t s);
 int pick_weight_shift(float absmax);
@@ -209,10 +217,10 @@
 enum LnMode { LN_PLAIN = 0, LN_AFFINE = 1, LN_ADA = 2 };
 void launch_layernorm_ch(const float* x, float* y, long bs, int ld, int C, LenMap len, int B, int Lmax,
                          float eps, int mode, const float* g, const float* be, int g_bs, float leaky,
-                         hipStream_t s);
+                         hipStream_t s, void* img = nullptr, long img_bs = 0, float img_prescale = 1.f);
 
 void launch_attention(const float* qkv, long bs, int ld, float* ctx, long cbs, int cld, const int* lens, int B,
-                      int Tmax, hipStream_t s);
+                      int Tmax, hipStream_t s, void* img = nullptr, long img_bs = 0, float img_prescale = 1.f, int img_only = 0);
 
 struct FcDesc {
     const float* w;
diff --git a/kokorox_amd/csrc/model.h b/kokorox_amd/csrc/model.h
--- a/kokorox_amd/csrc/model.h
+++ b/kokorox_amd/csrc/model.h
@@ -86,6 +86,9 @@
     int up_pad = 0, up_off = 0, up_reflect = 0;
     LenMap up_len{nullptr, 1, 0};
     float2* stat_part = nullptr;
+    void* img_out = nullptr;
+    float img_prescale = 1.f;
+    int img_only = 0;
 };
 
 std::vector<unsigned char> read_weight_file(const char* path, int* variant = nullptr);
@@ -174,6 +177,7 @@
     long fc_off(const std::string& key) const;
 
     void conv(const ConvW& w, const T& in, const T& out, const ConvOpts& o);
+    ConvPlan conv_plan_of(const ConvW& w, const T& in, const T& out, const ConvOpts& o, int x_image) const;
     void stats(const T& x, const std::string& fc_key);
     void adain_resblk(const std::string& name, const T& x, const T& out, bool upsample, float* ws_a, float* ws_b,
                       float* ws_c);
@@ -267,6 +271,9 @@
     struct PartInfo { const float2* part; int tiles, cols_per_tile, C; };
     std::map<const float*, PartInfo> parts_;
 
+    struct ImgInfo { void* img; long bs; int ld, C; float prescale; bool only; };
+    std::map<const float*, ImgInfo> imgs_;
+
     double call_ms_[4] = {0, 0, 0, 0};
     bool diag_on_ = false;
     std::vector<DiagRec> diag_recs_;
diff --git a/kokorox_amd/csrc/model.hip b/kokorox_amd/csrc/model.hip
--- a/kokorox_amd/csrc/model.hip
+++ b/kokorox_amd/csrc/model.hip
@@ -545,7 +545,7 @@
     }
 };
 
-void Model::conv(const ConvW& w, const T& in, const T& out, const ConvOpts& o) {
+ConvPlan Model::conv_plan_of(const ConvW& w, const T& in, const T& out, const ConvOpts& o, int x_image) const {
     const int prec1 = (conv_mode == CONV_F16 && p1_region_) ? 1 : ((conv_mode == CONV_BF16 && p1_region_ && w.w16b) ? 2 : 0);
     const void* w8x = conv_mode == CONV_F16F8 ? w.w8x : nullptr;
     ConvLaunch c{};
@@ -574,7 +574,25 @@
     c.B = B_;
     c.cols = (o.store == ST_UPSCATTER) ? in.Lmax + 1 : out.Lmax;
     c.cus = dry_ ? 0 : conv16_cu_count();
-    const ConvPlan plan = conv_plan(c);
+    c.x_image = x_image;
+    return conv_plan(c);
+}
+
+void Model::conv(const ConvW& w, const T& in, const T& out, const ConvOpts& o) {
+    const int prec1 = (conv_mode == CONV_F16 && p1_region_) ? 1 : ((conv_mode == CONV_BF16 && p1_region_ && w.w16b) ? 2 : 0);
+    const void* w8x = conv_mode == CONV_F16F8 ? w.w8x : nullptr;
+    ImgInfo xi{};
+    bool has_xi = false;
+    {
+        auto it = imgs_.find(in.p);
+        if (it != imgs_.end()) {
+            xi = it->second;
+            has_xi = xi.C == w.Cin && xi.ld == in.ld && xi.prescale == std::ldexp(1.0f, w.act_shift) && o.nmean == nullptr;
+            KX_REQUIRE(has_xi || !xi.only, "internal: a tensor that exists as an image only meets a reader that cannot take it");
+        }
+    }
+    const ConvPlan plan = conv_plan_of(w, in, out, o, has_xi);
+    KX_REQUIRE(plan.form == FORM_DAGI || !has_xi || !xi.only, "internal: a tensor that exists as an image only meets a launch of another form");
     void* x16 = nullptr;
     long x16_bs = 0;
     if (plan.pre) {
@@ -646,6 +664,20 @@
         diag_recs_.push_back(DiagRec{w.name, w.rows, w.Cin, w.K, w.act_shift, 0.0, 0.0, 0.0});
     }
     parts_.erase(out.p);
+    imgs_.erase(out.p);
+    if (plan.form == FORM_DAGI) {
+        a.x16 = xi.img;
+        a.x16_bs = xi.bs;
+        a.x16_ld = xi.ld;
+        if (o.img_out && o.store == ST_NORMAL && !o.accum && w.rows % 16 == 0) {
+            a.y16 = o.img_out;
+            a.y16_bs = (long)conv16_pre_image_bytes(w.rows, out.ld);
+            a.y16_ld = out.ld;
+            a.y16_prescale = o.img_prescale;
+            a.y16_only = o.img_only;
+            imgs_[out.p] = ImgInfo{o.img_out, a.y16_bs, out.ld, w.rows, o.img_prescale, o.img_only != 0};
+        }
+    }
     if (plan.stat_cols) {
         a.stat_part = o.stat_part;
         a.stat_tiles = plan.stat_tiles;
@@ -1199,6 +1231,7 @@
     taps_on_ = (flags & 2u) != 0;
     taps_.clear();
     parts_.clear();
+    imgs_.clear();
     p1_region_ = false;
     lane_ev_used_ = 0;
     prefix_keys_.clear();
@@ -1222,6 +1255,7 @@
         xchg_epoch_[0] = xchg_epoch_[1] = 0;
     }
 
+    void *h_img, *ctx_img, *av_img, *ff_img;
     float *emb, *h, *qkv, *ctx, *av, *ff, *dcat, *gxT, *gxT2, *xl, *logits, *te0, *te1, *t_en, *d_speeds;
     int *dur, *idx;
     auto planT = [&](Arena& A) {
@@ -1259,6 +1293,10 @@
         te0 = A.f(bt * 512);
         te1 = A.f(bt * 512);
         t_en = A.f(bt * 512);
+        h_img = A.alloc((size_t)B * conv16_pre_image_bytes(768, Tp));
+        ctx_img = A.alloc((size_t)B * conv16_pre_image_bytes(768, Tp));
+        av_img = A.alloc((size_t)B * conv16_pre_image_bytes(768, Tp));
+        ff_img = A.alloc((size_t)B * conv16_pre_image_bytes(2048, Tp));
     };
     arenaT_.measure = true;
     planT(arenaT_);
@@ -1318,23 +1356,43 @@
                         wt(E + "LayerNorm.bias"), 0, 0.f, stream_);
     tap("bert.emb", t_emb);
     conv(convs_.at("bert.map"), t_emb, t_h, ConvOpts{});
+    const ConvW &w_qkv = convs_.at("bert.qkv"), &w_dense = convs_.at("bert.dense"), &w_ffn = convs_.at("bert.ffn"),
+                &w_ffo = convs_.at("bert.ffn_out"), &w_benc = convs_.at("bert_encoder");
+    auto ps_of = [](const ConvW& w) { return std::ldexp(1.0f, w.act_shift); };
+    const long img768 = (long)conv16_pre_image_bytes(768, Tp);
+    ConvOpts od;
+    od.resid = &t_h;
+    ConvOpts of;
+    of.epi = EPI_GELU_NEW;
+    ConvOpts oo;
+    oo.resid = &t_a;
+    const bool images = conv_mode == CONV_F16X3 || conv_mode == CONV_F16F8;
+    const bool ctx_only = images && !taps_on_ && conv_plan_of(w_dense, t_ctx, t_a, od, 1).form == FORM_DAGI;
+    const bool ff_only = images && !taps_on_ && conv_plan_of(w_ffo, t_f, t_h, oo, 1).form == FORM_DAGI &&
+                         conv_plan_of(w_ffn, t_a, t_f, of, 1).form == FORM_DAGI;
+    of.img_out = images ? ff_img : nullptr;
+    of.img_prescale = ps_of(w_ffo);
+    of.img_only = ff_only;
     for (int l = 0; l < 12; ++l) {
-        conv(convs_.at("bert.qkv"), t_h, t_qkv, ConvOpts{});
-        launch_attention(qkv, t_qkv.bs, Tp, ctx, t_ctx.bs, Tp, dT_, B, Tmax, stream_);
-        ConvOpts od;
-        od.resid = &t_h;
-        conv(convs_.at("bert.dense"), t_ctx, t_a, od);
+        conv(w_qkv, t_h, t_qkv, ConvOpts{});
+        launch_attention(qkv, t_qkv.bs, Tp, ctx, t_ctx.bs, Tp, dT_, B, Tmax, stream_, images ? ctx_img : nullptr, img768, ps_of(w_dense),
+                         ctx_only);
+        imgs_.erase(ctx);
+        if (images) imgs_[ctx] = ImgInfo{ctx_img, img768, Tp, 768, ps_of(w_dense), ctx_only};
+        conv(w_dense, t_ctx, t_a, od);
         launch_layernorm_ch(av, av, t_a.bs, Tp, 768, LT, B, Tmax, 1e-12f, LN_AFFINE,
-                            wt(AL + "attention.LayerNorm.weight"), wt(AL + "attention.LayerNorm.bias"), 0, 0.f, stream_);
-        ConvOpts of;
-        of.epi = EPI_GELU_NEW;
-        conv(convs_.at("bert.ffn"), t_a, t_f, of);
-        ConvOpts oo;
-        oo.resid = &t_a;
-        conv(convs_.at("bert.ffn_out"), t_f, t_h, oo);
+                            wt(AL + "attention.LayerNorm.weight"), wt(AL + "attention.LayerNorm.bias"), 0, 0.f, stream_,
+                            images ? av_img : nullptr, img768, ps_of(w_ffn));
+        imgs_.erase(av);
+        if (images) imgs_[av] = ImgInfo{av_img, img768, Tp, 768, ps_of(w_ffn), false};
+        conv(w_ffn, t_a, t_f, of);
+        conv(w_ffo, t_f, t_h, oo);
+        const float ps_h = ps_of(l < 11 ? w_qkv : w_benc);
         launch_layernorm_ch(h, h, t_h.bs, Tp, 768, LT, B, Tmax, 1e-12f, LN_AFFINE,
                             wt(AL + "full_layer_layer_norm.weight"), wt(AL + "full_layer_layer_norm.bias"), 0, 0.f,
-                            stream_);
+                            stream_, images ? h_img : nullptr, img768, ps_h);
+        imgs_.erase(h);
+        if (images) imgs_[h] = ImgInfo{h_img, img768, Tp, 768, ps_h, false};
         if (l == 0) tap("bert.layer0", t_h);
     }
     tap("bert.out", t_h);
diff --git a/kokorox_amd/hip_koko.py b/kokorox_amd/hip_koko.py
--- a/kokorox_amd/hip_koko.py
+++ b/kokorox_amd/hip_koko.py
@@ -140,6 +140,9 @@
                                           i32, cp, sz]),
         "kx_test_lstm_parts": (i32, [i32]),
         "kx_test_conv_plan": (i32, [vp, i32, vp, i32, cp, sz]),
+        "kx_test_gemm_image": (i32, [i32, vp, vp, i32, i32, i32, vp, vp, i32, vp, i32, i32, i32, i32, i32, vp, vp, cp, sz]),
+        "kx_test_layernorm": (i32, [i32, vp, vp, i32, i32, i32, f32, i32, vp, vp, f32, i32, vp, vp, cp, sz]),
+        "kx_test_attention_image": (i32, [i32, vp, vp, i32, i32, i32, i32, vp, vp, cp, sz]),
     }
     for name, (res, args) in sig.items():
         fn = getattr(lib, name)
@@ -150,7 +153,8 @@
 
 
 TEST_ABI_SYMBOLS = ["kx_test_conv1d", "kx_test_lstm", "kx_test_source", "kx_test_attention", "kx_test_conv1d_epilogue", "kx_test_conv1d_full",
-                    "kx_test_conv_transpose", "kx_test_lstm_fault", "kx_test_lstm_parts", "kx_test_conv_plan"]
+                    "kx_test_conv_transpose", "kx_test_lstm_fault", "kx_test_lstm_parts", "kx_test_conv_plan", "kx_test_gemm_image",
+                    "kx_test_layernorm", "kx_test_attention_image"]
 
 ABI_SYMBOLS = [
     "kx_version", "kx_init", "kx_create", "kx_import_onnx", "kx_create_from_device_blob", "kx_create_replicas", "kx_replicas_times", "kx_create_partition", "kx_destroy",
@@ -572,10 +576,10 @@
 
 
 CONV_LAUNCH_FIELDS = ("mode", "prec1", "f8", "BM", "rows", "n_chunks16", "K", "dil", "stride", "pad", "act", "in_up2", "store", "accum",
-                      "epi", "norm", "stats", "image", "merge_T", "x_bs", "x_ld", "B", "cols", "cus", "force")
+                      "epi", "norm", "stats", "image", "merge_T", "x_bs", "x_ld", "B", "cols", "cus", "force", "x_image")
 CONV_PLAN_FIELDS = ("form", "bm", "act", "kt", "wm", "wn", "vt", "pf", "p1", "bf", "bn", "cols", "merged", "pre", "stat_cols",
                     "stat_tiles", "flat_bn")
-CONV_FORMS = ("F32", "LDS", "DAG", "DAGN", "DA", "DA_W2", "DA_S16", "DA_F8", "DA_PRE", "DAPN")
+CONV_FORMS = ("F32", "LDS", "DAG", "DAGN", "DA", "DA_W2", "DA_S16", "DA_F8", "DA_PRE", "DAPN", "DAGI")
 
 
 def conv_plan(**launch):
@@ -655,6 +659,66 @@
     return ctx
 
 
+def _image_shape(B, C, T):
+    return (B, (C + 15) // 16, 2, 2, (T + 31) // 32 * 32, 8)
+
+
+def split_image_ref(y, lens, shift=0):
+    y = np.asarray(y, dtype=np.float32)
+    B, Cc, T = y.shape
+    v = np.clip(y * np.float32(2.0 ** shift), np.float32(-65504.0), np.float32(65504.0)).astype(np.float32)
+    hi = v.astype(np.float16)
+    lo = (v - hi.astype(np.float32)).astype(np.float16)
+    img = np.zeros(_image_shape(B, Cc, T), dtype=np.uint16)
+    mask = np.zeros(img.shape, dtype=bool)
+    for pl, part in enumerate((hi, lo)):
+        pad = np.zeros((B, img.shape[1] * 16, T), dtype=np.float16)
+        pad[:, :Cc] = part
+        img[:, :, pl, :, :T, :] = pad.view(np.uint16).reshape(B, -1, 2, 8, T).transpose(0, 1, 2, 4, 3)
+    for b in range(B):
+        mask[b, :, :, :, :int(lens[b]), :] = True
+    return img, mask
+
+
+def gemm_image(x, lens, w, bias=None, resid=None, gelu=False, tmajor=False, x_shift=0, y_shift=0, fed=False, out_image=False,
+               only=False, merged=False, device=0):
+    lib = load_test_library()
+    x, w = _f32(x), _f32(w)
+    B, Cin, T = x.shape
+    Cout = w.shape[0]
+    lens = np.ascontiguousarray(np.asarray(lens, dtype=np.int32))
+    y = np.zeros((B, T, Cout) if tmajor else (B, Cout, T), dtype=np.float32)
+    img = np.zeros(_image_shape(B, Cout, T), dtype=np.uint16) if out_image else None
+    flags = (1 if fed else 0) | (2 if out_image else 0) | (4 if only else 0) | (8 if merged else 0)
+    _err_call(lib.kx_test_gemm_image, device, _ptr(x), _ptr(lens), B, Cin, T, _ptr(w), _ptr(_f32(bias)), Cout, _ptr(_f32(resid)),
+              1 if gelu else 0, 1 if tmajor else 0, x_shift, y_shift, flags, _ptr(y), _ptr(img))
+    return (y, img) if out_image else y
+
+
+def layernorm(x, lens, eps=1e-5, mode=0, g=None, be=None, leaky=0.0, image=False, img_shift=0, device=0):
+    lib = load_test_library()
+    x = _f32(x)
+    B, Cc, T = x.shape
+    lens = np.ascontiguousarray(np.asarray(lens, dtype=np.int32))
+    y = np.zeros_like(x)
+    img = np.zeros(_image_shape(B, Cc, T), dtype=np.uint16) if image else None
+    _err_call(lib.kx_test_layernorm, device, _ptr(x), _ptr(lens), B, Cc, T, float(eps), mode, _ptr(_f32(g)), _ptr(_f32(be)), float(leaky),
+              img_shift, _ptr(y), _ptr(img))
+    return (y, img) if image else y
+
+
+def attention_image(qkv, lens, img_shift=0, only=False, device=0):
+    lib = load_test_library()
+    qkv = _f32(qkv)
+    B, Cc, T = qkv.shape
+    assert Cc == 2304
+    lens = np.ascontiguousarray(np.asarray(lens, dtype=np.int32))
+    ctx = np.zeros((B, 768, T), dtype=np.float32)
+    img = np.zeros(_image_shape(B, 768, T), dtype=np.uint16)
+    _err_call(lib.kx_test_attention_image, device, _ptr(qkv), _ptr(lens), B, T, img_shift, 1 if only else 0, _ptr(ctx), _ptr(img))
+    return ctx, img
+
+
 def harmonic_source(f0, lin_w, lin_b, seed=0, utt_base=0, noise_off=False, device=0):
     lib = load_test_library()
     f0 = _f32(f0)
```

Measured after the change: 6905 x realtime (median of 6 runs). Within noise of the previous version (+0.4%).
